# Henning1/resql

Measured on AMD Instinct MI355X. Metric: TPC-H Q1 rows/s at SF10, higher is better.
Workload: dtype int64; 1 GPU; TPC-H Q1 over lineitem SF10 (59999996 rows, 7 columns, 38 B/row) resident in HBM, row-range sharded over 1 GPU(s); rows=59999996, rows_per_gpu=59999996, world_size=1, rccl_ranks_seen=1, backend=none (single process, single GPU), ranks=1, self_launched=False, parallelism=single GPU

## Files before the change

__graft_entry__.py:

```python
from __future__ import annotations

import os
import subprocess
import sys

ROOT = os.path.dirname(os.path.abspath(__file__))
if ROOT not in sys.path:
    sys.path.insert(0, ROOT)


def _prepopulate_kernel_cache() -> int:
    from resql_amd import engine, tpch
    ctx = engine.Context(device=-1)
    compiled = 0
    try:
        for plan in tpch.standard_plans(0.01):
            tabs = [ctx.table(t) for t in plan.tables]
            try:
                q = ctx.compile(plan, tabs)
                compiled += 1
                q.close()
            except engine.EngineError as e:
                if e.status != 3:
                    raise
# ... 103 lines not shown
                    continue
                os.environ.update(env, RSQ_DICT_SCANS="1")
                try:
                    tabs = [ctx.table(t) for t in (host if host is not None else stmt.tables)]
                    (ctx.sql_compile(stmt, tabs) if isinstance(stmt, str) else ctx.compile(stmt, tabs)).close()
                    for t in tabs:
                        t.close()
                    done += 1
                except engine.EngineError as e:
                    failed += e.status not in (2, 3)
                finally:
                    for k in list(env) + ["RSQ_DICT_SCANS"]:
                        os.environ.pop(k, None)
        elif kind == "dictjoin":
            import dictjoincases
            for i, (stmt, host, env) in enumerate(dictjoincases.warm_statements()):
                if i not in items:
                    continue
                for sw in ("2", "1", "0"):
                    if sw == "2":
                        os.environ.update(env)
                    os.environ["RSQ_DICT_SCANS"] = sw
                    try:
                        tabs = [ctx.table(t) for t in host]
                        (ctx.sql_compile(stmt, tabs) if isinstance(stmt, str) else ctx.compile(stmt, tabs)).close()
                        for t in tabs:
                            t.close()
                        done += 1
                    except engine.EngineError as e:
                        failed += e.status not in (2, 3)
                    finally:
                        for k in list(env) + ["RSQ_DICT_SCANS"]:
                            os.environ.pop(k, None)
        elif kind == "resulttext":
            import resulttextcases
            for i, (sql, host) in enumerate(resulttextcases.warm_statements()):
                if i not in items:
                    continue
                try:
                    tabs = [ctx.table(t) for t in host]
                    ctx.sql_compile(sql, tabs).close()
                    for t in tabs:
                        t.close()
                    done += 1
                except engine.EngineError as e:
                    failed += e.status not in (2, 3)
        else:
            if kind == "fuzz":
                import fuzzplans
                make = lambda s: fuzzplans.make(s)[0]
            else:
                import test_gpu_fuzz_joins
                make = lambda s: test_gpu_fuzz_joins.make(7000 + s)[0]
            for seed in items:
                try:
                    plan = make(seed)
                    tabs = [ctx.table(t) for t in plan.tables]
                    ctx.compile(plan, tabs).close()
                    for t in tabs:
                        t.close()
                    done += 1
                except engine.EngineError as e:
                    failed += e.status not in (2, 3)
    finally:
        ctx.close()
    return done, failed


def _prepopulate_test_kernels() -> int:
    import json
    n = max(1, min(16, os.cpu_count() or 1))
    jobs = []
    for kind, seeds in (("fuzz", list(range(320))), ("joins", list(range(120))), ("sql", list(range(45)) + list(range(200, 225))),
                        ("narrow", list(range(200))),
                        ("typed", list(range(32))),
                        ("ldsfold", list(range(32))),
                        ("dictgroup", list(range(64))),
                        ("dicttail", list(range(32))),
                        ("dictjoin", list(range(32))),
                        ("resulttext", list(range(32)))):
        for i in range(n):
            part = seeds[i::n]
            if part:
                jobs.append((kind, part))
    try:
        with open(os.path.join(ROOT, "tests", "golden", "sql_reference.json")) as f:
            gold = json.load(f)
        texts = [g["sql"] for g in gold["results"].values() if "refused" not in g]
        for i in range(n):
            if texts[i::n]:
                jobs.append(("sql", texts[i::n]))
    except Exception:
        pass
    import subprocess
    import time
    import signal
    deadline = time.time() + float(os.environ.get("RSQ_BUILD_WARM_SECONDS", "900"))
    env = dict(os.environ, RSQ_COMPILE_HELPERS="0")
    pending, running, done, failed, crashed = list(jobs), [], 0, 0, 0
    while pending or running:
        while pending and len(running) < n:
            kind, items = pending.pop()
            running.append(subprocess.Popen([sys.executable, os.path.abspath(__file__), "--warm", kind, json.dumps(items)], env=env,
                                            stdout=subprocess.PIPE, stderr=subprocess.DEVNULL, text=True, start_new_session=True))
        for pr in list(running):
            if pr.poll() is not None:
                out = pr.stdout.read().strip().split()
                if pr.returncode == 0 and len(out) >= 2 and out[-2].isdigit() and out[-1].isdigit():
                    done += int(out[-2]); failed += int(out[-1])
                else:
                    crashed += 1
                running.remove(pr)
        if time.time() > deadline:
# ... 108 lines not shown
```

include/resql_hip.h:

```cpp
#ifndef RESQL_HIP_H
#define RESQL_HIP_H

#include "resql_plan.h"

#ifdef __cplusplus
extern "C" {
#endif

typedef struct rsq_ctx   rsq_ctx;
typedef struct rsq_table rsq_table;
typedef struct rsq_query rsq_query;

enum rsq_status {
    RSQ_OK = 0,
    RSQ_ERR_INVALID = 1,
    RSQ_ERR_TYPE = 2,
    RSQ_ERR_UNSUPPORTED = 3,
    RSQ_ERR_DEVICE = 4,
    RSQ_ERR_RUNTIME = 5,
    RSQ_ERR_NOMEM = 6
};

typedef struct rsq_config {
    uint32_t struct_size;
// ... 137 lines not shown
int  rsq_query_report(const rsq_query* q, rsq_report* out);
int  rsq_query_kernel_time_stats(rsq_query* q, double* sum_ms, uint64_t* executions, int32_t reset);
int  rsq_query_nested_loops_slices(const rsq_query* q, int32_t* out);
#define RSQ_NLJ_MIN_SLICE_ROWS 512
int32_t rsq_nested_loops_slices(int64_t base_workgroups, int64_t max_workgroups, int64_t inner_rows, int32_t configured);
const char* rsq_query_source(const rsq_query* q);
const char* rsq_query_explain(const rsq_query* q);
void rsq_query_destroy(rsq_query* q);

char* rsq_serialize_expr(rsq_ctx* ctx, const rsq_plan_desc* plan, int32_t expr, int32_t derive,
                         rsq_table* const* tables, int32_t n_tables);
char* rsq_result_serialize(const rsq_result_view* view);
void  rsq_free(void* p);
typedef struct rsq_result_text_options {
    uint32_t struct_size;
    int32_t  mode;
    int64_t  chunk_rows;
    int64_t  max_device_bytes;
} rsq_result_text_options;
enum rsq_text_fallback { RSQ_TEXT_FALLBACK_NONE = 0, RSQ_TEXT_FALLBACK_NO_DEVICE = 1, RSQ_TEXT_FALLBACK_SCHEMA = 2, RSQ_TEXT_FALLBACK_DOES_NOT_FIT = 3 };
typedef struct rsq_result_text_report {
    uint32_t struct_size;
    int32_t  path;
    int32_t  fallback_reason;
    int32_t  tuples_from_device;
    int64_t  rows, text_bytes, chunks;
    double   upload_ms, kernel_ms, download_ms, total_ms;
} rsq_result_text_report;
int  rsq_query_result_text(rsq_query* q, const rsq_result_text_options* options , rsq_result_text_report* report ,
                           char** text, int64_t* text_bytes);
int  rsq_query_result_write(rsq_query* q, const char* path, const rsq_result_text_options* options, rsq_result_text_report* report);
int  rsq_ctx_set_result_text(rsq_ctx* ctx, int32_t where);
int  rsq_ctx_set_row_cells(rsq_ctx* ctx, int32_t mode);
int  rsq_ctx_set_order_limit(rsq_ctx* ctx, int32_t where);
enum rsq_order_limit_fallback { RSQ_ORDER_LIMIT_FALLBACK_NONE = 0, RSQ_ORDER_LIMIT_FALLBACK_SHAPE = 1, RSQ_ORDER_LIMIT_FALLBACK_FEW_ROWS = 2,
                                RSQ_ORDER_LIMIT_FALLBACK_OVERFLOW = 3, RSQ_ORDER_LIMIT_FALLBACK_TIES = 4 };
typedef struct rsq_order_limit_report {
    uint32_t struct_size;
    int32_t  planned;
    int32_t  path;
    int32_t  fallback_reason;
    int32_t  first_key_column;
    int32_t  key_is32;
    int32_t  descending;
    int32_t  reserved;
    int64_t  rows, want, candidates, capacity;
    double   select_ms, copy_ms, tail_ms;
} rsq_order_limit_report;
int  rsq_query_order_limit_report(const rsq_query* q, rsq_order_limit_report* out);
int   rsq_ref_emission_order(const uint64_t* hashes, int64_t n, uint64_t min_size, int32_t parallel, uint32_t* out);
int   rsq_ref_emission_order_device(rsq_ctx* ctx, const uint64_t* hashes, int64_t n, uint64_t min_size, uint32_t* out);

int   rsq_prim_exclusive_scan(rsq_ctx* ctx, const uint32_t* counts, int64_t n, int32_t form, uint64_t* offsets , uint32_t* notes);
int   rsq_prim_rank_index(rsq_ctx* ctx, uint32_t* blocks , int64_t n_blocks, int32_t form,
                          uint32_t* chunk_base , uint32_t* notes);
int   rsq_prim_rank_place(rsq_ctx* ctx, const uint32_t* blocks , int64_t n_blocks, int64_t bm_min, int64_t bm_bits,
                          const int64_t* records , const uint32_t* used , int32_t n_waves,
                          int32_t region, int32_t n_words, int64_t capacity, int64_t* words_out , uint32_t* notes);
int   rsq_prim_radix_sort_pairs(rsq_ctx* ctx, const uint64_t* keys , const uint32_t* vals , int64_t n, int32_t key_bits,
                                uint64_t* keys_out , uint32_t* vals_out , uint32_t* notes);
int   rsq_prim_running_min(rsq_ctx* ctx, const int64_t* in , int64_t n, int64_t* out , uint32_t* notes);
int   rsq_prim_merge_group_rows(rsq_ctx* ctx, const int64_t* rows , int64_t n, int32_t stride, int32_t n_tab,
                                const int32_t* key_word, const int32_t* key_type, const int32_t* key_len, int32_t n_keys, const int32_t* acc_word,
                                const int32_t* acc_kind, int32_t n_acc, int64_t* out_rows , uint64_t* out_count, uint32_t* notes);
int   rsq_prim_topk_select(rsq_ctx* ctx, const int64_t* rows , int64_t n_rows, int64_t rows_upper_bound, int32_t stride,
                           int32_t key_word, int32_t is32, int32_t desc, int64_t want, int32_t form, const uint64_t* image_range ,
                           int64_t capacity, int64_t* cand_out , uint32_t* cand_count, uint32_t* notes);
int   rsq_prim_column_topk(rsq_ctx* ctx, const void* key , int32_t key_width, int64_t n, int32_t desc, int64_t want,
                           int64_t capacity, const void* payload , int32_t payload_width,
                           uint32_t* positions_out , void* payload_out , uint64_t* cand_count,
                           uint64_t* threshold_image, uint32_t* notes);
int   rsq_table_read_image(rsq_ctx* ctx, const rsq_table* t, const char* column, int32_t which, void* host_dst, size_t bytes, int64_t info[4]);

typedef struct rsq_sql_plan rsq_sql_plan;
int  rsq_sql_plan_select(rsq_ctx* ctx, const char* sql, rsq_table* const* tables, int32_t n_tables, rsq_sql_plan** out);
const rsq_plan_desc* rsq_sql_plan_desc(const rsq_sql_plan* plan);
void rsq_sql_plan_destroy(rsq_sql_plan* plan);
char* rsq_sql_plan_text(const rsq_sql_plan* plan);
int  rsq_sql_compile(rsq_ctx* ctx, const char* sql, rsq_table* const* tables, int32_t n_tables, rsq_query** out);
char* rsq_sql_describe(rsq_ctx* ctx, const char* sql, int32_t what);

typedef struct rsq_db rsq_db;
int  rsq_db_create(rsq_ctx* ctx, rsq_db** out);
int  rsq_db_execute(rsq_db* db, const char* sql, int32_t* kind, rsq_result_view* result);
const char* rsq_db_message(const rsq_db* db);
int  rsq_db_adopt_table(rsq_db* db, rsq_table* table);
int  rsq_db_report(const rsq_db* db, rsq_report* out);
int  rsq_db_load_report(const rsq_db* db, rsq_tbl_load_report* out);
int  rsq_db_result_text_report(const rsq_db* db, rsq_result_text_report* out);
int  rsq_db_order_limit_report(const rsq_db* db, rsq_order_limit_report* out);
void rsq_db_destroy(rsq_db* db);

enum rsq_merge_mode { RSQ_MERGE_AUTO = 0, RSQ_MERGE_RCCL = 1, RSQ_MERGE_PEER_COPY = 2 };
typedef struct rsq_multi_config {
    uint32_t struct_size;
    int32_t n_devices;
    const rsq_config* base;
    const int32_t* devices;
    int32_t merge;
    int32_t reserved0;
} rsq_multi_config;
typedef struct rsq_multi rsq_multi;
typedef struct rsq_multi_query rsq_multi_query;
int  rsq_multi_create(const rsq_multi_config* cfg, rsq_multi** out);
void rsq_multi_destroy(rsq_multi* m);
// ... 25 lines not shown
```

integration/resql_hip_binding.h:

```cpp
#pragma once

#include <map>
#include <memory>
#include <string>
#include <vector>
#include <cstring>

#include "resql_hip.h"

namespace resql_hip {

struct HipError : public ResqlError {
    int status;
    HipError(int st, const std::string& m) : ResqlError(m), status(st) {}
};

inline rsq_type toRsqType(SqlType t) {
    rsq_type r{(int32_t)t.tag, 0, 0, 0};
    if (t.tag == SqlType::DECIMAL) { r.precision = t.decimalSpec().precision; r.scale = t.decimalSpec().scale; }
    if (t.tag == SqlType::CHAR) r.len = (int32_t)t.charSpec().num;
    if (t.tag == SqlType::VARCHAR) r.len = (int32_t)t.varcharSpec().num;
    return r;
}

// ... 120 lines not shown
        c.print_assembly = cfg.printAssembly; c.print_flounder = cfg.printFlounder; c.print_performance = cfg.printPerformance;
        c.num_threads = cfg.numThreads; c.emit_machine_code = cfg.emitMachineCode; c.optimize = cfg.optimizeFlounder;
        c.device = device;
        int rc = rsq_ctx_create(&c, &ctx_);
        if (rc != RSQ_OK) throw HipError(rc, rsq_last_error(nullptr));
        report.config = cfg;
    }
    ~JitContextHip() {
        for (auto& kv : tables_) rsq_table_destroy(kv.second.t);
        if (ctx_) rsq_ctx_destroy(ctx_);
    }

    rsq_table* deviceTable(Relation* rel, const std::string& name) {
        auto it = tables_.find(rel);
        if (it == tables_.end()) {
            Resident r;
            r.t = fromBlocks(rel, name, 0, 0);
            noteSynced(rel, r);
            tables_[rel] = r;
            return r.t;
        }
        Resident& r = it->second;
        if (r.deviceOnly || rel->tupleNum() == r.tuples) return r.t;
        if (rel->tupleNum() < r.tuples) throw ResqlError("Relation " + name + " holds fewer tuples than its device copy.");
        rsq_table* more = fromBlocks(rel, name, r.blocks ? r.blocks - 1 : 0, r.blocks ? r.lastBlockBytes : 0);
        int rc = rsq_table_append(r.t, more);
        if (rc != RSQ_OK) { rsq_table_destroy(more); check(rc); }
        noteSynced(rel, r);
        return r.t;
    }

    void setRowstoreBridge(int where) { check(rsq_ctx_set_rowstore_bridge(ctx_, where)); }
    void setOrderLimit(int where) { check(rsq_ctx_set_order_limit(ctx_, where)); }

    int64_t bulkInsert(Relation* rel, const std::string& name, const std::string& fileName, char fieldTerminator) {
        std::vector<rsq_column> cols = columnsOf(rel);
        rsq_table_desc d{};
        std::strncpy(d.name, name.c_str(), RSQ_SYMBOL_MAX - 1);
        d.n_cols = (int32_t)cols.size(); d.cols = cols.data();
        rsq_table* t = nullptr;
        check(rsq_table_load_tbl(ctx_, &d, fileName.c_str(), fieldTerminator, 0, &t));
        const int64_t inserted = rsq_table_rows(t);
        auto it = tables_.find(rel);
        if (it == tables_.end()) {
            if (rel->tupleNum() != 0) { rsq_table_destroy(t); throw ResqlError("Table " + name + " holds host tuples: BULK INSERT onto the device needs an empty or device-resident table."); }
            Resident r; r.t = t; r.deviceOnly = true;
            tables_[rel] = r;
        } else {
            int rc = rsq_table_append(it->second.t, t);
            if (rc != RSQ_OK) { rsq_table_destroy(t); check(rc); }
        }
        return inserted;
    }

    std::unique_ptr<Relation> run(RelOperator* root, bool requestAll) {
        PlanDescriber pd;
        bool hasLimit = false; int64_t limit = 0;
        int rootIdx = pd.op(root, &hasLimit, &limit);
        rsq_plan_desc plan{};
        plan.exprs = pd.exprs.data(); plan.n_exprs = (int32_t)pd.exprs.size();
        plan.ops = pd.ops.data(); plan.n_ops = (int32_t)pd.ops.size();
        plan.root = rootIdx; plan.request_all = requestAll ? 1 : 0;
        plan.has_limit = hasLimit ? 1 : 0; plan.limit = limit;
        std::vector<rsq_table*> tabs;
        for (size_t i = 0; i < pd.tables.size(); i++) tabs.push_back(deviceTable(pd.tables[i], pd.tableNames[i]));
        rsq_query* q = nullptr;
// ... 62 lines not shown
```

resql_amd/csrc/aot_kernels.hip:

```cpp
#include <hip/hip_runtime.h>

#include <algorithm>
#include <cstring>

#include "engine_internal.h"
#include "scan_device.h"

namespace rsq {

template <typename T>
__global__ void __launch_bounds__(256) k_minmax(const T* __restrict__ p, i64 n, i64* out ) {
    i64 mn = 0x7fffffffffffffffll, mx = (i64)0x8000000000000000ull;
    u64 desc = 0;
    u64 same = 0;
    for (i64 i = blockIdx.x * (i64)blockDim.x + threadIdx.x; i < n; i += (i64)gridDim.x * blockDim.x) {
        i64 v = (i64)p[i];
        mn = v < mn ? v : mn; mx = v > mx ? v : mx;
        if (i > 0) { const i64 pv = (i64)p[i - 1]; if (v < pv) desc++; if (v == pv) same++; }
    }
    for (int m = 32; m >= 1; m >>= 1) {
        i64 a = __shfl_xor(mn, m, 64), b = __shfl_xor(mx, m, 64);
        mn = a < mn ? a : mn; mx = b > mx ? b : mx;
        desc += (u64)__shfl_xor((long long)desc, m, 64);
        same += (u64)__shfl_xor((long long)same, m, 64);
    }
    if ((threadIdx.x & 63) == 0) {
        atomicMin(&out[0], mn); atomicMax(&out[1], mx);
        if (desc) atomicAdd(reinterpret_cast<u64*>(&out[2]), desc);
        if (same) atomicAdd(reinterpret_cast<u64*>(&out[3]), same);
    }
}

__global__ void __launch_bounds__(256) k_byteset(const unsigned char* __restrict__ p, i64 n, unsigned* out ) {
    __shared__ unsigned s[8];
    if (threadIdx.x < 8) s[threadIdx.x] = 0;
    __syncthreads();
    unsigned loc[8] = {0, 0, 0, 0, 0, 0, 0, 0};
    for (i64 i = blockIdx.x * (i64)blockDim.x + threadIdx.x; i < n; i += (i64)gridDim.x * blockDim.x) {
// ... 17 lines not shown
        if (c.type.tag == RSQ_BOOL || (c.type.tag == RSQ_CHAR && c.type.len == 1)) {
            bool seen[256] = {false};
            const unsigned char* p = (const unsigned char*)c.dptr;
            for (int64_t i = 0; i < t.nRows; i++) seen[p[i]] = true;
            for (int v = 0; v < 256; v++) if (seen[v]) c.stats.distinctBytes.push_back((uint8_t)v);
            c.stats.min = c.stats.distinctBytes.front(); c.stats.max = c.stats.distinctBytes.back();
            c.stats.valid = true;
        } else if (rangeStatsType(c.type)) {
            int64_t mn = INT64_MAX, mx = INT64_MIN, prev = INT64_MIN;
            bool asc = true, strict = true;
            for (int64_t i = 0; i < t.nRows; i++) {
                int64_t v = (w == 8) ? ((const int64_t*)c.dptr)[i]
                          : (c.type.tag == RSQ_DATE ? (int64_t)((const uint32_t*)c.dptr)[i] : (int64_t)((const int32_t*)c.dptr)[i]);
                mn = std::min(mn, v); mx = std::max(mx, v);
                if (v < prev) asc = false;
                if (i > 0 && v <= prev) strict = false;
                prev = v;
            }
            c.stats.min = mn; c.stats.max = mx; c.stats.valid = true; c.stats.ascending = asc; c.stats.strictlyAscending = asc && strict;
        }
    }
}

int narrowWidth(const TableColumn& c) {
    if (!sw::flag<sw::RSQ_NARROW_SCANS>()) return 0;
    if (!c.owned || !c.dptr || !c.stats.valid || c.type.isString()) return 0;
    const int tag = c.type.tag;
    if (tag != RSQ_INT && tag != RSQ_BIGINT && tag != RSQ_DECIMAL && tag != RSQ_DATE) return 0;
    if (c.stats.min == INT64_MIN || c.stats.max == INT64_MAX || c.stats.max < c.stats.min) return 0;
    const uint64_t range = (uint64_t)c.stats.max - (uint64_t)c.stats.min;
    const int w = range <= 0xffull ? 1 : range <= 0xffffull ? 2 : range <= 0xffffffffull ? 4 : 0;
    if (tag == RSQ_INT && w != 1) return 0;
    return w > 0 && w < columnWidth(c.type) ? w : 0;
}

enum { DICT_MAX = 256, DICT_SLOTS = 1024, DICT_SAMPLE_ROWS = 65536, DICT_COLLECT_GRID = 512 };

__device__ inline unsigned dictHash(const unsigned char* p, int W) {
    unsigned h = 2166136261u;
    for (int i = 0; i < W; i++) h = (h ^ p[i]) * 16777619u;
    return h;
}
__device__ inline bool dictSame(const unsigned char* a, const unsigned char* b, int W) {
    for (int i = 0; i < W; i++) if (a[i] != b[i]) return false;
    return true;
}

__global__ void __launch_bounds__(256) k_dict_collect(const unsigned char* __restrict__ col, i64 n, int W, const unsigned* __restrict__ countsIn,
                                                      unsigned char* __restrict__ out, unsigned* __restrict__ counts, unsigned* overflow) {
    __shared__ unsigned long long slot[DICT_SLOTS];
    __shared__ unsigned cnt, wpos;
    for (int i = threadIdx.x; i < DICT_SLOTS; i += 256) slot[i] = ~0ull;
    if (threadIdx.x == 0) { cnt = 0; wpos = 0; }
    __syncthreads();
    for (i64 base = (i64)blockIdx.x * 256; base < n; base += (i64)gridDim.x * 256) {
        if (*(volatile unsigned*)&cnt > (unsigned)DICT_MAX || *(volatile unsigned*)overflow) break;
        const i64 r = base + threadIdx.x;
        if (r >= n) continue;
        if (countsIn && (unsigned)(r & 255) >= countsIn[r >> 8]) continue;
        const unsigned char* v = col + r * W;
        unsigned h = dictHash(v, W) & (DICT_SLOTS - 1);
        for (int probe = 0; probe < DICT_SLOTS; probe++, h = (h + 1) & (DICT_SLOTS - 1)) {
            unsigned long long cur = *(volatile unsigned long long*)&slot[h];
            if (cur == ~0ull) {
                cur = atomicCAS(&slot[h], ~0ull, (unsigned long long)r);
                if (cur == ~0ull) { if (atomicAdd(&cnt, 1u) >= (unsigned)DICT_MAX) atomicExch(overflow, 1u); break; }
// ... 263 lines not shown
    TableColumn& c = t.cols[(size_t)col];
    if (ctx.device < 0 || c.dictN <= 0 || !c.codePtr || !c.dictPtr || t.nRows <= 0) failInvalid("column " + c.name + " of table " + t.name + " has no dictionary codes on a device");
    if (which != 0 && which != 1) failInvalid("dictionary pass: 0 (recode) or 1 (encode)");
    RSQ_HIP(hipSetDevice(ctx.device));
    unsigned char ident[256];
    for (int i = 0; i < 256; i++) ident[i] = (unsigned char)i;
    unsigned char* dLut = (unsigned char*)ctx.alloc(256 + 16);
    unsigned* dFlag = (unsigned*)(dLut + 256);
    float ms = 0;
    unsigned notFound = 0;
    try {
        RSQ_HIP(hipMemcpyAsync(dLut, ident, 256, hipMemcpyHostToDevice, ctx.stream));
        RSQ_HIP(hipMemsetAsync(dFlag, 0, sizeof(unsigned), ctx.stream));
        RSQ_HIP(hipEventRecord(ctx.ev0, ctx.stream));
        if (which == 0) {
            const i64 vectors = ((i64)t.nRows + 15) >> 4;
            hipLaunchKernelGGL(k_dict_recode, dim3((unsigned)std::min<i64>(2048, (vectors + 255) / 256)), dim3(256), 0, ctx.stream, (unsigned char*)c.codePtr, (i64)t.nRows,
                               (const unsigned char*)dLut);
        } else {
            hipLaunchKernelGGL(k_dict_encode, dim3((unsigned)std::min<int64_t>(2048, (t.nRows + 255) / 256)), dim3(256), 0, ctx.stream, (const unsigned char*)c.dptr, (i64)t.nRows,
                               columnWidth(c.type), (const unsigned char*)c.dictPtr, c.dictN, (unsigned char*)c.codePtr, dFlag);
        }
        RSQ_HIP(hipGetLastError());
        RSQ_HIP(hipEventRecord(ctx.ev1, ctx.stream));
        RSQ_HIP(hipMemcpyAsync(&notFound, dFlag, sizeof notFound, hipMemcpyDeviceToHost, ctx.stream));
        RSQ_HIP(hipStreamSynchronize(ctx.stream));
        RSQ_HIP(hipEventElapsedTime(&ms, ctx.ev0, ctx.ev1));
    } catch (...) { (void)hipStreamSynchronize(ctx.stream); ctx.free(dLut); throw; }
    ctx.free(dLut);
    if (notFound) throw Error(RSQ_ERR_DEVICE, "dictionary pass over table " + t.name + ": a row holds a value that is not in the column's dictionary");
    return (double)ms;
}

template <typename T, typename N>
__global__ void __launch_bounds__(256) k_encode(const T* __restrict__ src, N* __restrict__ dst, i64 n, i64 base) {
    for (i64 i = blockIdx.x * (i64)blockDim.x + threadIdx.x; i < n; i += (i64)gridDim.x * blockDim.x)
        dst[i] = (N)((u64)(i64)src[i] - (u64)base);
}

template <typename T>
static void launchEncode(Context& ctx, const TableColumn& c, i64 n) {
    const unsigned grid = 1024;
    if (c.nw == 1) hipLaunchKernelGGL((k_encode<T, unsigned char>), dim3(grid), dim3(256), 0, ctx.stream, (const T*)c.dptr, (unsigned char*)c.nptr, n, (i64)c.nbase);
    else if (c.nw == 2) hipLaunchKernelGGL((k_encode<T, unsigned short>), dim3(grid), dim3(256), 0, ctx.stream, (const T*)c.dptr, (unsigned short*)c.nptr, n, (i64)c.nbase);
    else hipLaunchKernelGGL((k_encode<T, unsigned>), dim3(grid), dim3(256), 0, ctx.stream, (const T*)c.dptr, (unsigned*)c.nptr, n, (i64)c.nbase);
}

static void buildNarrowImages(Context& ctx, Table& t) {
    bool moved = false, launched = false;
    for (auto& c : t.cols) {
        const int w = t.nRows > 0 ? narrowWidth(c) : 0;
        const int64_t base = w ? c.stats.min : 0;
        const size_t bytes = w ? (((size_t)t.nRows * (size_t)w + 15) & ~(size_t)15) : 0;
        const bool keep = ctx.device >= 0 && c.nptr && w == c.nw && base == c.nbase && bytes == c.nbytes;
        if (!keep && c.nptr) { if (ctx.device >= 0) { ctx.freeRaw(c.nptr); ctx.columnImageBytes -= c.nbytes; } c.nptr = nullptr; moved = true; }
        c.nw = w; c.nbase = base; c.nbytes = bytes;
        if (!w || ctx.device < 0) continue;
        if (!c.nptr) { c.nptr = ctx.allocRaw(bytes); ctx.columnImageBytes += bytes; }
        launched = true;
        if (c.type.tag == RSQ_INT) launchEncode<int>(ctx, c, (i64)t.nRows);
        else if (c.type.tag == RSQ_DATE) launchEncode<unsigned>(ctx, c, (i64)t.nRows);
        else launchEncode<i64>(ctx, c, (i64)t.nRows);
    }
    if (launched) { RSQ_HIP(hipGetLastError()); RSQ_HIP(hipStreamSynchronize(ctx.stream)); }
    if (moved) t.layoutVersion++;
    buildDictImages(ctx, t);
}

void computeColumnStats(Context& ctx, Table& t) {
    if (ctx.device < 0) { hostStats(t); buildNarrowImages(ctx, t); return; }
    if (t.nRows == 0) {
        for (auto& c : t.cols) c.stats = ColumnStats();
        buildNarrowImages(ctx, t);
        return;
    }
    RSQ_HIP(hipSetDevice(ctx.device));
    i64* dmm = (i64*)ctx.alloc(4 * sizeof(i64));
    unsigned* dset = (unsigned*)ctx.alloc(8 * sizeof(unsigned));
    const unsigned grid = 1024;
    for (auto& c : t.cols) {
        c.stats = ColumnStats();
        if (!c.dptr) continue;
        if (c.type.tag == RSQ_BOOL || (c.type.tag == RSQ_CHAR && c.type.len == 1)) {
// ... 1357 lines not shown
```

resql_amd/csrc/api.cpp:

```cpp
#include <algorithm>
#include <chrono>
#include <cstdlib>
#include <cstring>
#include <map>
#include <thread>

#include "engine.h"
#include "sqlfront.h"
#include "hostref.h"

using namespace rsq;

namespace {
thread_local std::string g_createError;

template <typename F>
int guarded(Context* ctx, F&& f) {
    try { f(); return RSQ_OK; }
    catch (const Error& e) { if (ctx) ctx->lastError = e.what(); else g_createError = e.what(); return e.status; }
    catch (const std::bad_alloc&) { if (ctx) ctx->lastError = "out of host memory"; return RSQ_ERR_NOMEM; }
    catch (const std::exception& e) { if (ctx) ctx->lastError = e.what(); else g_createError = e.what(); return RSQ_ERR_INVALID; }
}

Context* C(rsq_ctx* c) { return reinterpret_cast<Context*>(c); }
// ... 405 lines not shown
    if (!ctx || !t || !name || !host_dst) return RSQ_ERR_INVALID;
    return guarded(C(ctx), [&] {
        const Table* tb = reinterpret_cast<const Table*>(t);
        int ci = tb->findCol(name);
        if (ci < 0 || !tb->cols[(size_t)ci].dptr) failInvalid(std::string("no such column: ") + name);
        size_t have = (size_t)tb->nRows * (size_t)columnWidth(tb->cols[(size_t)ci].type);
        if (bytes > have) failInvalid("read beyond the column");
        if (C(ctx)->device >= 0) RSQ_HIP(hipMemcpy(host_dst, tb->cols[(size_t)ci].dptr, bytes, hipMemcpyDeviceToHost));
        else memcpy(host_dst, tb->cols[(size_t)ci].dptr, bytes);
    });
}

int rsq_table_read_image(rsq_ctx* ctx, const rsq_table* t, const char* name, int32_t which, void* host_dst, size_t bytes, int64_t info[4]) {
    if (!ctx || !t || !name || !info || which < 0 || which > 2 || (bytes && !host_dst)) return RSQ_ERR_INVALID;
    return guarded(C(ctx), [&] {
        const Table* tb = reinterpret_cast<const Table*>(t);
        if (tb->ctx != C(ctx)) failInvalid("the table belongs to another context");
        int ci = tb->findCol(name);
        if (ci < 0) failInvalid(std::string("no such column: ") + name);
        const TableColumn& c = tb->cols[(size_t)ci];
        info[0] = c.nw; info[1] = c.nw ? c.nbase : 0; info[2] = c.dictN; info[3] = tb->nRows;
        if (!bytes) return;
        const bool device = C(ctx)->device >= 0;
        if (!device && which != 1) failUnsupported("a compile-only context keeps no narrow image and no dictionary codes");
        const size_t have = which == 0 ? (size_t)tb->nRows * (size_t)c.nw
                          : which == 1 ? (size_t)c.dictN * (size_t)columnWidth(c.type)
                                       : (c.dictN ? (size_t)tb->nRows : 0);
        if (bytes > have) failInvalid("read beyond the image");
        if (!device) { memcpy(host_dst, c.dict.data(), bytes); return; }
        const void* src = which == 0 ? c.nptr : which == 1 ? c.dictPtr : c.codePtr;
        if (!src) failInvalid("the column has no such image");
        RSQ_HIP(hipStreamSynchronize(C(ctx)->stream));
        RSQ_HIP(hipMemcpy(host_dst, src, bytes, hipMemcpyDeviceToHost));
    });
}

void rsq_table_destroy(rsq_table* t) { delete T(t); }

int rsq_query_compile(rsq_ctx* ctx, const rsq_plan_desc* plan, rsq_table* const* tables, int32_t n_tables, rsq_query** out) {
    if (!ctx || !plan || !out || n_tables < 0) return RSQ_ERR_INVALID;
    *out = nullptr;
    return guarded(C(ctx), [&] {
        std::unique_ptr<QueryHandle> h(new QueryHandle{C(ctx), nullptr});
        h->q = compileQuery(*C(ctx), *plan, tables, n_tables);
        *out = reinterpret_cast<rsq_query*>(h.release());
    });
}

#define QH(q) reinterpret_cast<QueryHandle*>(q)

int rsq_query_execute(rsq_query* q) {
    if (!q) return RSQ_ERR_INVALID;
    return guarded(QH(q)->ctx, [&] { executeQuery(*QH(q)->q, false); });
}

int rsq_query_await_kernels(rsq_query* q) {
    if (!q) return RSQ_ERR_INVALID;
    return guarded(QH(q)->ctx, [&] { awaitKernels(*QH(q)->q); });
}

int rsq_query_execute_partial(rsq_query* q, void** dev_ptr, int64_t* n_min_words, int64_t* n_max_words, int64_t* n_sum_words) {
    if (!q || !dev_ptr || !n_min_words || !n_max_words || !n_sum_words) return RSQ_ERR_INVALID;
    return guarded(QH(q)->ctx, [&] {
        executeQuery(*QH(q)->q, true);
        partialBuffer(*QH(q)->q, dev_ptr, n_min_words, n_max_words, n_sum_words);
    });
// ... 852 lines not shown
```

resql_amd/csrc/codegen.cpp:

```cpp
#include "codegen_internal.h"

namespace rsq {
namespace cg {

void Walker::addArg(const std::string& name, const std::string& ctype, uint64_t v) {
    for (auto& a : pipe.args) if (a.name == name) return;
    pipe.args.push_back({name, ctype, v});
}

void Walker::produce(OpNode* o, std::vector<std::string> request) {
    switch (o->tag) {
        case RSQ_OP_SCAN: produceScan(o, request); break;
        case RSQ_OP_SELECTION: {
            o->schema.clear();
            std::vector<std::string> r = request;
            requiredAttributes(o->exprs[0], r);
            requestOf[o] = request;
            produce(o->child[0], r);
            break;
        }
        case RSQ_OP_PROJECTION: {
            std::vector<std::string> r;
            for (Expr* e : o->exprs) requiredAttributes(e, r);
            produce(o->child[0], r);
            break;
        }
        case RSQ_OP_HASHJOIN: {
            requestOf[o] = request;
            std::vector<std::string> all = request;
            for (Expr* e : o->exprs) requiredAttributes(e, all);
            joinPhase[o] = 1;
            produce(o->child[0], all);
            joinPhase[o] = 2;
            produce(o->child[1], all);
            break;
        }
        case RSQ_OP_AGGREGATION: {
            if (q.agg) failUnsupported("more than one aggregation in a plan");
            q.agg = o;
            std::vector<std::string> r;
// ... 135 lines not shown
        for (auto& b : numeric) line(b.ct + " " + b.var + "_b[" + Bs + "]; rsq::nlj_ld_block<" + b.ct + ", " + Bs + ">(a." + b.cn + ", " + N + "_jb, " + b.var + "_b);");
        line("#pragma unroll");
        openScope("for (int " + N + "_u = 0; " + N + "_u < " + Bs + "; " + N + "_u++) {");
        line("const i64 " + N + "_j = " + N + "_jb + " + N + "_u;");
        body += pairDeep.substr(0, pairDeep.find('\n') + 1);
        for (auto& b : numeric) line("const " + b.ct + " " + b.var + " = " + b.var + "_b[" + N + "_u];");
        body += pairDeep.substr(pairDeep.find('\n') + 1);
        closeScope();
        closeScope();
        openScope("for (i64 " + N + "_j = " + N + "_jb; " + N + "_j != " + hi + "; " + N + "_j++) {");
        body += pairFlat.substr(0, pairFlat.find('\n') + 1);
        singleLoads();
        body += pairFlat.substr(pairFlat.find('\n') + 1);
        closeScope();
    }
    closeScope();
}

Schema Walker::prune(const Schema& s, const std::vector<std::string>& req) {
    Schema r;
    for (auto& a : s) if (has(req, a.name)) r.push_back(a);
    return r;
}

void Walker::produceScan(OpNode* o, std::vector<std::string> request) {
    Table* t = o->table;
    if (o->derived >= 0) nameDerivedColumns(q, o);
    if (q.requestAll) request.clear();
    pipe = Pipeline();
    pipe.src = t;
    pipe.unroll = 1;
    pipe.blockThreads = 256;
    pipe.maxGrid = q.maxGrid;
    colTypes.clear(); colIsString.clear(); colNarrow.clear(); colDict.clear(); colTyped.clear(); eg.typedLeaves.clear(); nDictTables = 0; rowParams.clear(); rowArgsTail.clear(); rowArgsTailGuarded.clear(); bitmapPrefetch.clear();
    body.clear(); stateDecl.clear(); stateInit.clear(); prologue.clear(); epilogue.clear(); fileScope.clear(); helperFns.clear();
    explainSteps.clear(); indent = 1; matchSlotTable = -1; slotVar.clear(); symbolOrigin.clear(); symbolWord.clear();
    multiMatchAbove = false; repeatedKeysAbove.clear(); denseRefusal.clear();
    selective = false; compacted = false; stage2Body.clear(); cqLive.clear();
    leadCond.clear(); leadCols.clear(); leadPass = 1.0; leadPassComplete = true;
    pairSplit = std::string::npos; pairCond.clear();
    strPrefetch.clear(); strPrefetchWidth.clear(); strStaged.clear(); strStagedBytes = 0; postTile.clear(); foldTile.clear(); accRegs = 0; eg.strWordVars.clear();
    eg.symbols.clear();
    o->schema.clear();
    const bool narrowScans = sw::flag<sw::RSQ_NARROW_SCANS>();
    for (size_t ci = 0; ci < t->cols.size(); ci++) {
        const TableColumn& c = t->cols[ci];
        if (!request.empty() && !has(request, c.name)) continue;
        if (!c.dptr && !t->derived) {
            if (request.empty()) continue;
            failInvalid("column " + c.name + " is needed by the plan but was declared without data");
        }
        int k = (int)pipe.cols.size();
        pipe.cols.push_back((int)ci);
        std::string var = "v_" + std::to_string(k);
        eg.symbols[c.name] = Sym{var, c.type};
        symbolOrigin[c.name] = -1;
        o->schema.push_back({c.name, c.type});
        pipe.bytesPerRow += columnWidth(c.type);
        const int nw = (!t->derived && c.owned && narrowScans && !c.type.isString() && (c.nptr || q.ctx.device < 0)) ? c.nw : 0;
        colNarrow.push_back(nw);
        const bool dictCoded = !t->derived && c.owned && c.type.isString() && c.dictN > 0 && sw::dictScansEnabled() && (c.codePtr || q.ctx.device < 0);
        colDict.push_back(dictCoded ? c.type.len : 0);
        pipe.storedBytesPerRow += dictCoded ? 1 : nw ? nw : columnWidth(c.type);
        if (dictCoded) {
            const std::string K = std::to_string(k);
            addArg("c" + K, "const u8*", (uint64_t)(uintptr_t)c.codePtr);
            addArg("d" + K, "const char*", (uint64_t)(uintptr_t)c.dictPtr);
            addArg("dn" + K, "i64", (uint64_t)c.dictN);
            colIsString.push_back(0); colTypes.push_back("u8");
            rowParams += ", u8 vc_" + K;
            rowArgsTail += ", a.c" + K + "[r]";
            rowArgsTailGuarded += ", (valid ? a.c" + K + "[r] : (u8)0)";
            line("const rsq::Str " + var + " = " + dictDecode(k, "vc_" + K) + ";");
        } else if (c.type.isString()) {
            addArg("c" + std::to_string(k), "const char*", (uint64_t)(uintptr_t)c.dptr);
            colIsString.push_back(1); colTypes.push_back("");
            line("const rsq::Str " + var + " = rsq::str(a.c" + std::to_string(k) + " + lr * " + std::to_string(c.type.len) + ", " +
                 std::to_string(c.type.len) + ");");
        } else {
            std::string ct = ExprGen::ctype(c.type);
            if (nw) {
                addArg("c" + std::to_string(k), std::string("const ") + (nw == 1 ? "u8" : nw == 2 ? "u16" : "u32") + "*", (uint64_t)(uintptr_t)c.nptr);
                addArg("fb" + std::to_string(k), "i64", (uint64_t)c.nbase);
            } else addArg("c" + std::to_string(k), "const " + ct + "*", (uint64_t)(uintptr_t)c.dptr);
            colIsString.push_back(0); colTypes.push_back(ct);
            rowParams += ", " + ct + " " + var;
            rowArgsTail += ", " + colAt(k, "r");
            rowArgsTailGuarded += ", (valid ? " + colAt(k, "r") + " : (" + ct + ")0)";
        }
    }
    explainSteps.push_back("scan " + t->name + " [" + (t->derived ? std::string("rows of this execution") : std::to_string((long long)t->nRows) + " rows") + ", " +
                           std::to_string((long long)pipe.bytesPerRow) + " B/row" +
                           (pipe.storedBytesPerRow != pipe.bytesPerRow ? ", " + std::to_string((long long)pipe.storedBytesPerRow) + " B/row stored" : std::string()) + "]");
    consume(o->parent, o);
    finishPipeline();
}

bool Walker::sideRange(const Expr* e, double& lo, double& hi, int& col) {
    if (e->tag == RSQ_E_TYPECAST && e->child) {
        if (!sideRange(e->child, lo, hi, col)) return false;
        const int ds = (e->type.tag == RSQ_DECIMAL ? e->type.scale : 0) - (e->child->type.tag == RSQ_DECIMAL ? e->child->type.scale : 0);
        const double f = std::pow(10.0, (double)ds);
        lo *= f; hi *= f;
        return true;
    }
    auto linear = [&](double v) -> double {
        if (e->type.tag != RSQ_DATE) return v;
        const int64_t d = (int64_t)v;
        return (double)((d / 10000) * 372 + ((d / 100) % 100 - 1) * 31 + (d % 100 - 1));
    };
    if (e->tag == RSQ_E_CONSTANT && !e->type.isString()) { lo = hi = linear((double)e->ival); col = -1; return true; }
    if ((e->tag == RSQ_E_ADD || e->tag == RSQ_E_SUB) && e->child && e->child->next && e->type.tag != RSQ_DATE) {
        double alo, ahi, blo, bhi; int ac = -1, bc = -1;
        if (!sideRange(e->child, alo, ahi, ac) || !sideRange(e->child->next, blo, bhi, bc) || ac >= 0 || bc >= 0) return false;
        const int s0 = e->type.tag == RSQ_DECIMAL ? e->type.scale : 0;
        const double fa = std::pow(10.0, (double)(s0 - (e->child->type.tag == RSQ_DECIMAL ? e->child->type.scale : 0)));
        const double fb = std::pow(10.0, (double)(s0 - (e->child->next->type.tag == RSQ_DECIMAL ? e->child->next->type.scale : 0)));
        lo = hi = e->tag == RSQ_E_ADD ? alo * fa + blo * fb : alo * fa - blo * fb; col = -1;
        return true;
    }
    if (e->tag == RSQ_E_ATTRIBUTE) {
        auto so = symbolOrigin.find(e->symbol);
        if (so == symbolOrigin.end() || so->second != -1) return false;
        const int ci = pipe.src->findCol(e->symbol);
        if (ci < 0 || !pipe.src->cols[(size_t)ci].stats.valid || pipe.src->cols[(size_t)ci].type.isString()) return false;
        lo = linear((double)pipe.src->cols[(size_t)ci].stats.min); hi = linear((double)pipe.src->cols[(size_t)ci].stats.max); col = ci;
// ... 344 lines not shown
```

resql_amd/csrc/codegen_agg.cpp:

```cpp
#include "codegen_internal.h"
#include "row_cells.h"

namespace rsq {
namespace cg {

void Walker::collectAccumulators(OpNode* o) {
    for (Expr* g : o->exprs2) q.pool.addId(g);
    for (Expr* s : o->splitAgg) q.pool.addId(s);
    q.accums.clear(); q.splitToAccum.clear();
    q.accums.push_back(Accum{RSQ_E_MIN, "#firstrow", "row", Type(RSQ_BIGINT), 2});
    for (Expr* s : o->splitAgg) {
        Accum ac; ac.kind = s->tag; ac.type = s->type;
        dictTablesWithin(s);
        switch (s->tag) {
            case RSQ_E_COUNT: ac.key = "COUNT"; ac.input = eg.emit(s); ac.merge = 0; ac.inputExpr = nullptr; break;
            case RSQ_E_SUM:
                if (s->type.tag != RSQ_DECIMAL && s->type.tag != RSQ_BIGINT) failType("ADD code generation not implemented for datatype");
                ac.key = "SUM" + structuralKey(s->child); ac.input = eg.emit(s); ac.merge = 0; ac.inputExpr = s->child; break;
            case RSQ_E_MIN: case RSQ_E_MAX:
                if (s->type.tag != RSQ_DECIMAL && s->type.tag != RSQ_BIGINT && s->type.tag != RSQ_DATE)
                    failType(s->tag == RSQ_E_MAX ? "ADD code generation not implemented for datatype" : "LESS_THAN code generation not implemented for datatype");
                ac.key = std::string(s->tag == RSQ_E_MIN ? "MIN" : "MAX") + structuralKey(s->child);
                ac.input = "((i64)(" + eg.emit(s) + "))"; ac.merge = s->tag == RSQ_E_MIN ? 2 : 3; ac.inputExpr = s->child; break;
            default: failType("Aggregation type not implemented in updateAggregates(..).");
// ... 684 lines not shown
    for (int w = 1; w < W; w++) k << (w > 1 ? " : " : "") << (w < W - 1 ? "w == " + std::to_string(w) + " ? " : "") << "(i64)" << q.accumSlot[(size_t)w];
    k << ";\n        if (g < " << D << ") a.out[blk * " << D << " + g] = s_tab[i];\n    }\n}\n";
    pipe.sourceStagedAgg = k.str();
}

bool Walker::envelopeOf(const TableColumn& c, bool& neg, int& bits) {
    if (!c.owned || !c.stats.valid || c.stats.min <= -(int64_t(1) << 40) || c.stats.max >= (int64_t(1) << 40)) return false;
    const uint64_t m = (uint64_t)std::max(c.stats.max < 0 ? -c.stats.max : c.stats.max, c.stats.min < 0 ? -c.stats.min : c.stats.min);
    bits = 0;
    while (bits < 63 && (m >> bits) != 0) bits++;
    neg = c.stats.min < 0;
    return true;
}

bool Walker::typeScanColumns() {
    if (!sw::flag<sw::RSQ_NARROW_SCANS>() || compacted || !pipe.src || pipe.src->derived) return false;
    colTyped.assign(colTypes.size(), 0);
    std::string widen;
    for (size_t k = 0; k < colTypes.size(); k++) {
        if (colIsString[k] || coded((int)k) || !colNarrow[k] || colTypes[k] != "i64") continue;
        bool neg = false; int bits = 0;
        if (!envelopeOf(pipe.src->cols[(size_t)pipe.cols[k]], neg, bits) || bits > 31) continue;
        const std::string K = std::to_string(k);
        auto patch = [&](std::string& text, const std::string& from, const std::string& to) {
            for (size_t at = 0; (at = text.find(from, at)) != std::string::npos; at += to.size()) {
                const size_t end = at + from.size();
                if (isdigit((unsigned char)from.back()) && end < text.size() && isdigit((unsigned char)text[end])) { at = end - to.size(); continue; }
                text.replace(at, from.size(), to);
            }
        };
        patch(rowParams, ", i64 v_" + K, ", i32 n_" + K);
        patch(rowArgsTail, "rsq::dec<i64>(a.c" + K + "[", "rsq::dec<i32>(a.c" + K + "[");
        patch(rowArgsTailGuarded, "rsq::dec<i64>(a.c" + K + "[", "rsq::dec<i32>(a.c" + K + "[");
        colTyped[k] = 1; colTypes[k] = "i32";
        eg.typedLeaves["v_" + K] = ExprGen::TypedLeaf{"n_" + K, neg, bits};
        widen += "    const i64 v_" + K + " = (i64)n_" + K + "; (void)v_" + K + ";\n";
    }
    if (widen.empty()) return false;
    body = widen + body;
    return true;
}

void Walker::emitDenseAggregation(OpNode* o) {
    const int64_t D = q.denseGroups;
    const int W = (int)q.accums.size();
    line("const int gid = " + groupIdExpr() + ";");
    const bool typed = q.aggMode == AggMode::DENSE_REG && typeScanColumns();
    auto emitInputs = [&](const std::vector<char>& part32) {
        for (int w = 1; w < W; w++) {
            const Accum& ac = q.accums[(size_t)w];
            const std::string name = "in" + std::to_string(w);
            if (typed && ac.merge == 0 && ac.inputExpr && eg.pureArithmetic(ac.inputExpr)) {
                const ExprGen::TV v = eg.emitTyped(ac.inputExpr);
                if (v.is32 && part32[(size_t)w]) line("const i32 " + name + " = " + v.text + ";");
                else line("const i64 " + name + " = " + ExprGen::wide(v) + ";");
            } else line("const i64 " + name + " = " + ac.input + ";");
        }
    };
    if (q.aggMode != AggMode::DENSE_REG) emitInputs(std::vector<char>((size_t)W, 0));
    const bool fr32 = typed && !underNestedLoops() && pipe.src->nRows < (int64_t)0xffffffffll && pipe.src->totalRows() < (int64_t)0xffffffffll;
    auto inOf = [&](int w) { return w == 0 ? std::string("row") : "in" + std::to_string(w); };
    addArg("out", "u64*", 0);
    std::ostringstream ep;
    if (q.aggMode == AggMode::DENSE_REG) {
        std::vector<char> part32((size_t)W, 0);
        std::vector<rowcells::Accumulator> envelopes((size_t)W, rowcells::Accumulator{false, false, -1});
// ... 335 lines not shown
```

resql_amd/csrc/codegen_internal.h:

```cpp
#pragma once
#include <algorithm>
#include <cmath>
#include <cstring>
#include <functional>
#include <set>
#include <sstream>

#include "engine_internal.h"


namespace rsq {
namespace cg {


struct Sym { std::string var; Type type; };


struct ExprGen {
    std::map<std::string, Sym> symbols;
    std::map<std::string, int> strWordVars;
    bool int16Cast = false;
    std::map<const Expr*, std::string> tabled;

    static std::string ctype(const Type& t) {
// ... 258 lines not shown
            close += ")";
        }
        if (c) out += "(" + emit(c) + ")";
        else out += (e->type.isString() ? std::string("rsq::str(\"\", 0)") : "((" + ctype(e->type) + ")0)");
        return out + close;
    }
};

inline std::string fromWord(const std::string& w, const Type& t) {
    switch (t.tag) {
        case RSQ_BIGINT: case RSQ_DECIMAL: return w;
        case RSQ_INT: case RSQ_DATE: return "((i32)(" + w + "))";
        case RSQ_BOOL: return "((u8)(" + w + "))";
        case RSQ_CHAR: if (t.len == 1) return "((u8)(" + w + "))"; [[fallthrough]];
        case RSQ_VARCHAR: return "rsq::str_from_addr(" + w + ", " + std::to_string(t.len) + ")";
        default: failUnsupported("value type cannot be carried in a hash table word");
    }
}
inline std::string toWord(const std::string& v, const Type& t) {
    if (t.isString()) return "rsq::str_addr(" + v + ")";
    return "((i64)(" + v + "))";
}

struct Walker {
    Query& q;
    ExprGen eg;

    Pipeline pipe;
    std::vector<std::string> colTypes;
    std::vector<int> colIsString;
    std::vector<int> colNarrow;
    std::string colAt(int k, const std::string& r) const {
        const std::string K = std::to_string(k);
        if (k < (int)colNarrow.size() && colNarrow[(size_t)k]) return "rsq::dec<" + colTypes[(size_t)k] + ">(a.c" + K + "[" + r + "], a.fb" + K + ")";
        return "a.c" + K + "[" + r + "]";
    }
    std::string tileLoad(int k, const std::string& dst) const {
        const std::string K = std::to_string(k);
        if (k < (int)colNarrow.size() && colNarrow[(size_t)k]) return "rsq::ld2n(a.c" + K + " + b, a.fb" + K + ", " + dst + ");";
        return "rsq::ld2(a.c" + K + " + b, " + dst + ");";
    }
    std::vector<int> colDict;
    std::vector<char> colTyped;
    bool typedCol(int k) const { return k >= 0 && k < (int)colTyped.size() && colTyped[(size_t)k] != 0; }
    static bool envelopeOf(const TableColumn& c, bool& neg, int& bits);
    bool typeScanColumns();
    bool coded(int k) const { return k >= 0 && k < (int)colDict.size() && colDict[(size_t)k] != 0; }
    std::string paramName(int k) const { return (coded(k) ? "vc_" : typedCol(k) ? "n_" : "v_") + std::to_string(k); }
    std::string dictDecode(int k, const std::string& code) const {
        const std::string K = std::to_string(k), W = std::to_string(colDict[(size_t)k]);
        return "rsq::str(a.d" + K + " + (u32)(" + code + ") * " + W + "u, " + W + ")";
    }
    int nDictTables = 0;
    int dictTableColumn(const Expr* e, int col = -1);
    void dictTablesWithin(Expr* e);
    int storedWidth(int k) const {
        if (k < (int)colNarrow.size() && colNarrow[(size_t)k]) return colNarrow[(size_t)k];
        return colTypes[(size_t)k] == "i64" ? 8 : colTypes[(size_t)k] == "i32" ? 4 : 1;
    }
    std::string rowParams, rowArgsTail, rowArgsTailGuarded;
    struct BitmapPrefetch { std::string first; int second; bool interleaved; };
    std::vector<BitmapPrefetch> bitmapPrefetch;
    std::string body;
    std::string closers;
    std::string stateDecl, stateInit, prologue, epilogue, fileScope;
    std::string helperFns;
    std::vector<std::string> explainSteps;
    int indent = 1;
    int matchSlotTable = -1;
    std::map<int, std::string> slotVar;
    std::map<std::string, int> symbolOrigin;
    std::map<std::string, int> symbolWord;
    bool multiMatchAbove = false;
    std::string repeatedKeysAbove;
    std::string denseRefusal;
    bool underNestedLoops() const { return !q.nljs.empty(); }
    bool selective = false, compacted = false;
    std::string leadCond; std::vector<int> leadCols; double leadPass = 1.0;
    std::string stage2Prefix;
    struct CompFilter { std::string table, symbol, stage2Var; int64_t bits; };
    std::vector<CompFilter> compFilters;
    bool inStage2 = false;
    bool leadPassComplete = true;
    size_t pairSplit = std::string::npos; std::string pairCond;
    std::string stage2Body;
    std::vector<std::pair<std::string, Sym>> cqLive;

    explicit Walker(Query& q_) : q(q_) { eg.int16Cast = jitInt16Cast(q_.ctx); }

    void line(const std::string& s) { body += std::string((size_t)indent * 4, ' ') + s + "\n"; }
    void openScope(const std::string& head) { line(head); indent++; }
    void closeScope() { indent--; line("}"); }
    void addArg(const std::string& name, const std::string& ctype, uint64_t v);

    void produce(OpNode* o, std::vector<std::string> request);

    std::map<OpNode*, std::vector<std::string>> requestOf;
    std::map<OpNode*, int> joinPhase;

    static bool has(const std::vector<std::string>& v, const std::string& s) { return std::find(v.begin(), v.end(), s) != v.end(); }

    Schema prune(const Schema& s, const std::vector<std::string>& req);

    void produceScan(OpNode* o, std::vector<std::string> request);

    bool sideRange(const Expr* e, double& lo, double& hi, int& col);
    double passFraction(const Expr* e);
    void leadColumnsOf(const Expr* e, std::vector<int>& out, bool& ok);
    std::vector<std::pair<int, int>> strPrefetch;
    std::map<int, int> strPrefetchWidth;
    std::string foldTile;
    int accRegs = 0;
    bool rowCells = false;
    static constexpr const char* RC_IFNOT = "\x01rc-ifnot\n"; static constexpr const char* RC_IF = "\x01rc-if\n";
    static constexpr const char* RC_ELSE = "\x01rc-else\n"; static constexpr const char* RC_END = "\x01rc-end\n";
    static void resolveRowCells(std::string& text, bool keep);
    std::string postTile;
    std::map<int, int> strStaged;
    int strStagedBytes = 0;
    void prefetchComparedStrings(const Expr* e);
    void noteLeadingSelection(const Expr* e, const std::string& cond);

    void consume(OpNode* o, OpNode* from);

    bool downstreamMaterializes(OpNode* o);
    bool compactThen(OpNode* o, const std::function<void()>& downstream);
// ... 79 lines not shown
```

resql_amd/csrc/codegen_loop.cpp:

```cpp
#include "codegen_internal.h"

namespace rsq {
namespace cg {

std::string Walker::postTileFor(const std::string& tile) {
    std::string out = postTile;
    for (size_t at; (at = out.find("$TILE")) != std::string::npos;) out.replace(at, 5, tile);
    return out;
}

void Walker::stagedChunkLoads(std::ostringstream& s, const std::string& ind, const char* pre, int col, int u) {
    const int W = strPrefetchWidth[col];
    for (int r = 0; r < stagedRounds(col); r++)
        s << ind << pre << col << "_" << u << "_" << r << " = rsq::ld_str_chunk<" << W << ", " << r << ">(a.c" << col << " + (b - lane * 2) * " << W << ", lane);\n";
}

void Walker::stagedUnstage(std::ostringstream& s, const std::string& ind, int u) {
    for (auto& sp : strPrefetch) {
        auto it = strStaged.find(sp.first);
        if (it == strStaged.end()) continue;
        const int W = strPrefetchWidth[sp.first];
        for (int r = 0; r < stagedRounds(sp.first); r++)
            s << ind << "rsq::st_str_chunk<" << W << ", " << r << ">(strt + " << it->second << ", lane, q" << sp.first << "_" << u << "_" << r << ");\n";
    }
// ... 9 lines not shown
    }
    if (!strStaged.empty()) s << ind << "rsq::wave_lds_order();\n";
}

void Walker::emitLateLoads(std::ostringstream& s, const std::string& tile, int u, const std::vector<char>& lateCol, const std::string& tileEnd) {
    s << "        if (" << tile << " < " << tileEnd << ") {\n";
    for (int j = 0; j < 2; j++) {
        s << "            const bool lp" << j << " = lead_pred(a";
        for (int k : leadCols) s << ", t" << k << "_" << u << "[" << j << "]";
        s << ");\n";
    }
    s << "            if (lp0 | lp1) {\n                const i64 b = ((" << tile << ") << 7) + lane * 2;\n";
    for (size_t k = 0; k < lateCol.size(); k++) if (lateCol[k]) s << "                " << tileLoad((int)k, "t" + std::to_string(k) + "_" + std::to_string(u)) << "\n";
    s << "            }\n        }\n";
}

void Walker::resolveRowCells(std::string& text, bool keep) {
    std::string out;
    bool drop = false;
    for (size_t at = 0; at < text.size();) {
        size_t end = text.find('\n', at);
        end = end == std::string::npos ? text.size() : end + 1;
        const std::string ln = text.substr(at, end - at);
        at = end;
        if (ln == RC_IFNOT) { if (keep) out += "#if !RSQ_ROW_CELLS\n"; }
        else if (ln == RC_IF) { if (keep) out += "#if RSQ_ROW_CELLS\n"; else drop = true; }
        else if (ln == RC_ELSE) { if (keep) out += "#else\n"; else drop = true; }
        else if (ln == RC_END) { if (keep) out += "#endif\n"; drop = false; }
        else if (!drop) out += ln;
    }
    text = out;
}

void Walker::finishPipeline() {
    while (indent > 1) closeScope();
    addArg("n_rows", "i64", (uint64_t)pipe.src->nRows);
    addArg("row0", "i64", (uint64_t)pipe.src->row0);
    addArg("err", "u32*", (uint64_t)(uintptr_t)q.ctx.dErr);
    if (pipe.gridPerCU == 2 && pipe.storedBytesPerRow > 0)
        pipe.unroll = (int)std::max<int64_t>(1, std::min<int64_t>(foldTile.empty() ? 4 : 2, (4608 + pipe.storedBytesPerRow * 128 - 1) / (pipe.storedBytesPerRow * 128)));
    if (pipe.compact) pipe.unroll = 4;
    const bool mat = pipe.sink == SinkKind::MATERIALIZE;
    std::ostringstream s;
    s << "// generated by resql_amd/csrc/codegen.cpp\n//   ";
    for (size_t i = 0; i < explainSteps.size(); i++) {
        std::string step = explainSteps[i];
        const size_t lb = step.find(" [");
        if (step.compare(0, 5, "scan ") == 0 && lb != std::string::npos) step = step.substr(0, lb);
        const size_t kb = step.find(", key bitmap of ");
        if (kb != std::string::npos) {
            const size_t ke = step.find(" bits", kb);
            if (ke != std::string::npos) step = step.substr(0, kb) + ", key bitmap" + step.substr(ke + 5);
        }
        s << (i ? " -> " : "") << step;
    }
    s << "\n";
    if (1) s << "#define RSQ_NT_LOADS 1\n";
    s << "#include \"rsq_device.h\"\n";
    s << fileScope;
    if (nDictTables) {
        s << "__shared__ u64 s_dt[" << 4 * nDictTables << "];      // truth tables over dictionary-coded columns: 256 bits each, filled in the kernel's prologue\n";
        prologue += "    __syncthreads();\n";
        pipe.extraLdsBytes += 32 * nDictTables;
    }
    const bool cq = pipe.compact;
    const bool dbgStamps = sw::num<sw::RSQ_DEBUG_TAIL>() != 0 && !(pipe.sink == SinkKind::AGGREGATE && q.aggMode == AggMode::DENSE_REG);
    if (dbgStamps) addArg("dbg", "u64*", 0);
    if (pipe.staged && (cq || mat || !bitmapPrefetch.empty() || !pipe.lazyCols.empty() ||
// ... 38 lines not shown
        if (fourWaves) { pipe.unroll = u; pipe.gridPerCU = 4; }
    }
    rowCells = rowCells && fourWaves && pipe.sink == SinkKind::AGGREGATE;
    for (std::string* text : {&stateDecl, &prologue, &body, &foldTile, &epilogue}) resolveRowCells(*text, rowCells);
    if (!rowCells) pipe.rowCellsEnvelopes.clear();
    const int U = pipe.unroll;
    if (strStagedBytes > 0) {
        pipe.extraLdsBytes += (pipe.blockThreads / 64) * strStagedBytes;
        prologue += "    __shared__ __attribute__((aligned(16))) char s_strt[(RSQ_BLOCK_THREADS / 64) * " + std::to_string(strStagedBytes) + "];\n    char* const strt = s_strt + (threadIdx.x >> 6) * " +
                    std::to_string(strStagedBytes) + ";\n";
    }
    const int NV = 1 + pipe.compactWords;
    const bool queuesLimit = (144 * 1024) / std::max(1, (pipe.blockThreads / 64) * NV * 192 * 8 + pipe.extraLdsBytes) < 4;
    const int QCAP = (queuesLimit ? 128 : 192);
    const int NVL = 1 + pipe.compactWordsLazy;
    const bool twoForms = !pipe.lazyCols.empty();
    if (cq) {
        const int ldsPerWG = (pipe.blockThreads / 64) * NV * QCAP * 8 + pipe.extraLdsBytes;
        const int ldsPerWGLazy = (pipe.blockThreads / 64) * NVL * QCAP * 8 + pipe.extraLdsBytes;
        const int wgCap = pipe.unroll >= 3 ? 6 : 8;
        pipe.gridPerCU = std::max(2, std::min(wgCap, (144 * 1024) / std::max(1, ldsPerWG)));
        pipe.gridPerCULazy = std::max(2, std::min(wgCap, (144 * 1024) / std::max(1, ldsPerWGLazy)));
        stateDecl += "    int cq_n = 0;\n    u32 cq_rows = 0;\n    i64* cq;\n";
        addArg("cq_total", "unsigned long long*", 0);
        epilogue += "    if (blockIdx.x < 64) {\n        const u64 v = rsq::wave_sum((u64)st.cq_rows);\n        if ((threadIdx.x & 63) == 0 && v) atomicAdd(a.cq_total, (unsigned long long)v);\n    }\n";
        const std::string nv = twoForms ? "RSQ_CQ_NV" : std::to_string(NV);
        prologue += "    __shared__ i64 s_cq[(RSQ_BLOCK_THREADS / 64) * " + nv + " * " + std::to_string(QCAP) + "];\n";
        prologue += "    st.cq = s_cq + (threadIdx.x >> 6) * " + nv + " * " + std::to_string(QCAP) + ";\n";
    }
    if (twoForms) s << "#if RSQ_LAZY\n#define RSQ_CQ_NV " << NVL << "\n#else\n#define RSQ_CQ_NV " << NV << "\n#endif\n";
    s << "#ifndef RSQ_BLOCK_THREADS\n#define RSQ_BLOCK_THREADS " << pipe.blockThreads << "\n#endif\n";
    if (fourWaves) s << "#define RSQ_MIN_WG 4\n";
    s << "struct Args {\n";
    for (auto& a : pipe.args) s << "    " << a.ctype << " " << a.name << ";\n";
    s << "};\nstruct State {\n" << stateDecl << "};\n";
    s << helperFns;
    if (cq) {
        s << "#ifdef RSQ_STAGE2_CALL\nstatic __device__ __attribute__((noinline)) void stage2(const Args& a, State& st, const i64 row";
        for (int k = 0; k < pipe.compactWords; k++) s << ", const i64 qw_" << k;
        s << ")\n#else\n";
        s << "static RSQ_DEV void stage2(const Args& a, State& st, const i64 row";
        for (int k = 0; k < pipe.compactWords; k++) s << ", const i64 qw_" << k;
        s << ")\n#endif\n{\n" << stage2Body << "}\n";
        pipe.hasStage2 = true;
        s << "static RSQ_DEV void cq_drain(const Args& a, State& st, const int count) {\n";
        s << "    const int lane = threadIdx.x & 63;\n    const int i = st.cq_n - count + lane;\n    rsq::wave_lds_order();      // (the entries were pushed by other lanes)\n";
        s << "    if (lane < count) {\n        stage2(a, st, st.cq[i]";
        for (int k = 0; k < pipe.compactWordsLazy; k++) s << ", st.cq[" << (k + 1) * QCAP << " + i]";
        if (pipe.compactWords > pipe.compactWordsLazy) {
            s << "\n#if RSQ_LAZY\n            ";
            for (int k = pipe.compactWordsLazy; k < pipe.compactWords; k++) s << ", 0";
            s << "\n#else\n            ";
            for (int k = pipe.compactWordsLazy; k < pipe.compactWords; k++) s << ", st.cq[" << (k + 1) * QCAP << " + i]";
            s << "\n#endif\n        ";
        }
        s << ");\n        st.cq_rows++;\n    }\n    st.cq_n -= count;\n}\n";
    }
    if (late) {
        s << "static RSQ_DEV bool lead_pred(const Args& a";
        for (int k : leadCols) s << ", " << colTypes[(size_t)k] << " " << paramName(k);
        s << ") { ";
        for (int k : leadCols) if (coded(k)) s << "const rsq::Str v_" << k << " = " << dictDecode(k, paramName(k)) << "; (void)v_" << k << "; ";
        for (int k : leadCols) if (typedCol(k)) s << "const i64 v_" << k << " = (i64)n_" << k << "; ";
        s << "return " << leadCond << "; }\n";
    }
    if (pipe.staged) s << "#if RSQ_AGG_VARIANT == 3\ntemplate <int SP_SLOT>       // the row's place among the rows a thread handles per round\n#endif\n";
    s << "static RSQ_DEV void row_fn(const Args& a, State& st, const i64 lr" << (cq ? ", const bool valid" : "") << rowParams << ") {\n";
// ... 265 lines not shown
        const bool eagerOk = cqPipelined && eagerRegs * U <= budget, lazyOk = cqPipelined && lazyRegs * U <= budget;
        if (latePipelined || regPipelined || (eagerOk && (lazyOk || pipe.lazyCols.empty()))) emitPipelinedLoop();
        else if (lazyOk && !pipe.lazyCols.empty()) { s << "#if RSQ_LAZY\n"; emitPipelinedLoop(); s << "#else\n"; emitPlainLoop(); s << "#endif\n"; }
        else emitPlainLoop();
    }
    if (dbgStamps) s << "    if (a.dbg && threadIdx.x == 0) a.dbg[(u64)blockIdx.x * 8 + 1] = (u64)wall_clock64();\n";
    if (!postTile.empty()) s << "    st.in_tile = false;\n";
    if (cq) {
        s << "    for (i64 rb = (ntiles << 7) + (i64)" << bx << " * blockDim.x; rb < a.n_rows; rb += (i64)" << gx << " * blockDim.x) {\n";
        s << "        const i64 r = rb + threadIdx.x;\n        const bool valid = r < a.n_rows;\n";
        s << "        row_fn(a, st, r, valid" << rowArgsTailGuarded << ");\n";
        s << "        while (st.cq_n >= 64) cq_drain(a, st, 64);\n    }\n";
        s << "    while (st.cq_n > 0) cq_drain(a, st, st.cq_n < 64 ? st.cq_n : 64);\n";
    } else {
        if (mat) {
            s << "    for (i64 rb = (ntiles << 7) + (i64)blockIdx.x * blockDim.x + (i64)(threadIdx.x & ~63u); rb < a.n_rows; rb += (i64)gridDim.x * blockDim.x) {\n";
            s << "        const i64 r = rb + lane;\n        const bool valid = r < a.n_rows;\n";
            s << "        const i64 ttile = ntiles + ((rb - (ntiles << 7)) >> 6);\n        const i64 slot = ttile * 64 + lane;\n";
            s << "#if RSQ_PASS == 2\n        st.pos = a.toffs[ttile] + (u64)rsq::wave_excl_sum_u32(valid ? a.cnt[slot] : 0u);\n#endif\n";
            s << "        if (valid) row_fn(a, st, r" << rowArgsTail << ");\n";
            s << "#if RSQ_PASS == 1\n        a.cnt[slot] = st.cnt;\n        { const u32 ts = (u32)rsq::wave_sum((u64)st.cnt); if (lane == 0) a.tcnt[ttile] = ts; }\n        st.cnt = 0;\n#endif\n";
            s << "    }\n";
        } else {
        s << "    for (i64 r = (ntiles << 7) + (i64)" << bx << " * blockDim.x + threadIdx.x; r < a.n_rows; r += (i64)" << gx << " * blockDim.x) {\n";
        s << "        row_fn(a, st, r" << rowArgsTail << ");\n";
        s << "    }\n";
        }
    }
    if (pipe.staged) s << "#endif\n";
    if (dbgStamps) s << "    if (a.dbg && threadIdx.x == 0) a.dbg[(u64)blockIdx.x * 8 + 2] = (u64)wall_clock64();\n";
    s << epilogue;
    if (dbgStamps) s << "    __syncthreads();\n    if (a.dbg && threadIdx.x == 0) a.dbg[(u64)blockIdx.x * 8 + 3] = (u64)wall_clock64();\n";
    s << "}\n";
    pipe.source = s.str();
    if (!pipe.lazyCols.empty()) pipe.source = "#define RSQ_LAZY 0\n" + pipe.source;
    if (mat) {
        pipe.sourcePass1 = "#define RSQ_PASS 1\n" + pipe.source;
        pipe.source = "#define RSQ_PASS 2\n" + pipe.source;
    }
    if (q.aggPad > 1 && pipe.sink == SinkKind::AGGREGATE && !pipe.partitioned) {
        pipe.sourceFlat = "#define RSQ_OUT_STRIDE 1\n" + pipe.source;
        pipe.source = "#define RSQ_OUT_STRIDE " + std::to_string(q.aggPad) + "\n" + pipe.source;
    }
    if (rowCells) {
        const std::string guard = "#ifndef RSQ_ROW_CELLS\n#define RSQ_ROW_CELLS 0\n#endif\n";
        pipe.sourceCells = "#define RSQ_ROW_CELLS 1\n" + guard + pipe.source;
        pipe.source = guard + pipe.source;
        if (!pipe.sourceFlat.empty()) { pipe.sourceFlatCells = "#define RSQ_ROW_CELLS 1\n" + guard + pipe.sourceFlat; pipe.sourceFlat = guard + pipe.sourceFlat; }
    }
    if (pipe.partitioned) {
        pipe.sourcePartCount = "#define RSQ_AGG_VARIANT 1\n#define RSQ_BLOCK_THREADS 1024\n" + pipe.source;
        pipe.sourcePartScatter = "#define RSQ_AGG_VARIANT 2\n#define RSQ_BLOCK_THREADS 1024\n" + pipe.source;
        if (pipe.staged) pipe.sourceStagedScatter = "#define RSQ_AGG_VARIANT 3\n#define RSQ_BLOCK_THREADS 1024\n" + pipe.source;
        pipe.source = "#define RSQ_AGG_VARIANT 0\n" + pipe.source;
    }
    if (!pipe.lazyCols.empty()) {
        pipe.sourceLazy = pipe.source;
        const std::string off = "#define RSQ_LAZY 0\n";
        const size_t at = pipe.sourceLazy.find(off);
        if (at == std::string::npos) pipe.sourceLazy.clear();
        else {
            const int minWg = 0;
            pipe.sourceLazy.replace(at, off.size(), "#define RSQ_LAZY 1\n" + (minWg ? "#define RSQ_MIN_WG " + std::to_string(minWg) + "\n" : std::string()));
        }
    }
    std::string ex = "pipeline " + std::to_string(q.pipelines.size()) + ": ";
    for (size_t i = 0; i < explainSteps.size(); i++) ex += (i ? " -> " : "") + explainSteps[i];
// ... 14 lines not shown
```

resql_amd/csrc/engine.cpp:

```cpp
#include <algorithm>
#include <atomic>
#include <chrono>
#include <cstring>
#include <functional>
#include <sstream>

#include "engine_internal.h"

namespace rsq {

namespace {

uint64_t inverseOdd64(uint64_t a) { uint64_t x = a; for (int i = 0; i < 6; i++) x *= 2 - a * x; return x; }

void buildOps(Query& q, const rsq_plan_desc& p) {
    int extra = 0;
    for (int i = 0; i < p.n_ops; i++) if (p.ops[i].tag == RSQ_OP_ORDERBY) extra++;
    for (int i = 0; i < p.n_ops + extra; i++) q.ops.emplace_back(new OpNode());
    int nextExtra = p.n_ops;
    for (int i = 0; i < p.n_ops; i++) {
        const rsq_op& d = p.ops[i];
        OpNode* o = q.ops[(size_t)i].get();
        o->tag = d.tag;
        if (d.n_exprs < 0 || d.n_exprs > RSQ_MAX_OP_EXPRS || d.n_exprs2 < 0 || d.n_exprs2 > RSQ_MAX_OP_EXPRS) failInvalid("bad expression count");
// ... 173 lines not shown
        for (int64_t g = 0; g < D; g++) init[(size_t)(q.accumSlot[w] * D + g)] = idv;
    }
    q.dAgg = (uint64_t*)q.ctx.alloc(words * 8);
    q.dAggInit = (uint64_t*)q.ctx.alloc(words * 8);
    RSQ_HIP(hipMemcpy(q.dAggInit, init.data(), words * 8, hipMemcpyHostToDevice));
    q.hAgg.assign(words, 0);
    q.pinnedWords = words;
    q.tableWords = words;
    if (q.aggPad > 1) {
        q.padWords = words * (size_t)q.aggPad;
        std::vector<uint64_t> pinit(q.padWords + 1, 0);
        for (size_t i = 0; i < words; i++) pinit[i * (size_t)q.aggPad] = init[i];
        q.dAggWork = (uint64_t*)q.ctx.alloc((q.padWords + 1) * 8);
        q.dAggWorkInit = (uint64_t*)q.ctx.alloc((q.padWords + 1) * 8);
        RSQ_HIP(hipMemcpy(q.dAggWorkInit, pinit.data(), (q.padWords + 1) * 8, hipMemcpyHostToDevice));
        q.pinnedWords = q.padWords;
    }
}

std::string tierSource(const Pipeline& p, const std::string& source, bool quick) {
    return quick && p.hasStage2 ? "#define RSQ_STAGE2_CALL 1\n" + source : source;
}
static std::vector<std::string> kernelSources(const Query& q, bool quick = false) {
    std::vector<std::string> v;
    for (auto& p : q.pipelines) {
        auto T = [&](const std::string& s) { return tierSource(p, s, quick); };
        if (!p.sourcePass1.empty()) v.push_back(T(p.sourcePass1));
        if (!p.sourceFlat.empty()) v.push_back(T(p.sourceFlat));
        if (p.partitioned) { v.push_back(T(p.sourcePartCount)); v.push_back(T(p.sourcePartScatter)); v.push_back(p.sourcePartAgg); }
        if (p.staged) { v.push_back(T(p.sourceStagedScatter)); v.push_back(p.sourceStagedAgg); }
        v.push_back(T(p.source));
        if (!p.sourceCells.empty()) v.push_back(T(p.sourceCells));
        if (!p.sourceFlatCells.empty()) v.push_back(T(p.sourceFlatCells));
        if (!p.sourceLazy.empty()) v.push_back(T(p.sourceLazy));
        if (p.ldsSlots > 64 && q.aggMode == AggMode::HASH && p.sink == SinkKind::AGGREGATE && q.aggTable >= 0) {
            v.push_back(T("#define RSQ_LC_SLOTS 64\n" + p.source));
            if (!p.sourceLazy.empty()) v.push_back(T("#define RSQ_LC_SLOTS 64\n" + p.sourceLazy));
        }
    }
    return v;
}
static void resolveKernels(Query& q, bool quick = false) {
    Context& ctx = q.ctx;
    ctx.compileManyToCache(kernelSources(q, quick));
    q.quickTier = quick;
    for (auto& p : q.pipelines) {
        auto T = [&](const std::string& s) { return tierSource(p, s, quick); };
        p.fewGroupKernels.clear();
        if (!p.sourcePass1.empty()) p.kernelPass1 = &ctx.getKernel(T(p.sourcePass1), p.entry);
        if (!p.sourceFlat.empty()) p.kernelFlat = &ctx.getKernel(T(p.sourceFlat), p.entry);
        if (p.partitioned) {
            p.kernelPartCount = &ctx.getKernel(T(p.sourcePartCount), p.entry);
            p.kernelPartScatter = &ctx.getKernel(T(p.sourcePartScatter), p.entry);
            p.kernelPartAgg = &ctx.getKernel(p.sourcePartAgg, "rsq_part_agg");
        }
        if (p.staged) {
            p.kernelStagedScatter = &ctx.getKernel(T(p.sourceStagedScatter), p.entry);
            p.kernelStagedAgg = &ctx.getKernel(p.sourceStagedAgg, "rsq_staged_agg");
        }
        p.kernel = &ctx.getKernel(T(p.source), p.entry);
        if (!p.sourceCells.empty()) p.kernelCells = &ctx.getKernel(T(p.sourceCells), p.entry);
        if (!p.sourceFlatCells.empty()) p.kernelFlatCells = &ctx.getKernel(T(p.sourceFlatCells), p.entry);
        if (!p.sourceLazy.empty()) p.kernelLazy = &ctx.getKernel(T(p.sourceLazy), p.entry);
        if (ctx.device < 0 && p.ldsSlots > 64 && q.aggMode == AggMode::HASH && p.sink == SinkKind::AGGREGATE && q.aggTable >= 0) {
            (void)ctx.getKernel("#define RSQ_LC_SLOTS 64\n" + p.source, p.entry);
            if (!p.sourceLazy.empty()) (void)ctx.getKernel("#define RSQ_LC_SLOTS 64\n" + p.sourceLazy, p.entry);
        }
    }
}


static uint64_t fnv1a64(const std::string& s, uint64_t h = 1469598103934665603ull) {
    for (unsigned char c : s) { h ^= c; h *= 1099511628211ull; }
    return h;
}
static std::string planMemoKey(const Query& q) {
    uint64_t h = 1469598103934665603ull;
    for (auto& p : q.pipelines) h = fnv1a64(p.source, h) * 0x9E3779B97F4A7C15ull;
    std::string k = std::to_string(h);
    if (q.maxGrid) k += "|g" + std::to_string(q.maxGrid);
    for (Table* t : q.tables) k += "|" + std::to_string(t->uid) + "." + std::to_string(t->version) + "." + std::to_string(t->nRows) + "." + std::to_string(t->row0) + "." + std::to_string(t->nRowsTotal);
    return k;
}

static void applyPlanMemo(Query& q) {
    Context& ctx = q.ctx;
    if (ctx.planMemoOff || ctx.device < 0 || q.genericActive) return;
    if (!q.derived.empty()) return;
    q.memoKey = planMemoKey(q);
    auto it = ctx.planMemo.find(q.memoKey);
    if (it == ctx.planMemo.end()) return;
    Context::PlanMemo& m = it->second;
    if (m.joins.size() != q.hashTables.size() || m.pipes.size() != q.pipelines.size()) return;
    m.stamp = ++ctx.planMemoClock;
    for (size_t i = 0; i < q.pipelines.size(); i++) {
// ... 1550 lines not shown
```

resql_amd/csrc/engine.h:

```cpp
#pragma once

#include <hip/hip_runtime.h>

#include <atomic>
#include <cstdint>
#include <cstdio>
#include <cstdlib>
#include <functional>
#include <map>
#include <tuple>
#include <memory>
#include <mutex>
#include <set>
#include <string>
#include <vector>

#include "expr.h"
#include "hostref.h"
#include "mempool.h"
#include "resql_hip.h"
#include "rowstore.h"
#include "switches.h"
#include "tbl.h"

#define RSQ_RANK_CHUNK_BLOCKS 1024

namespace rsq {

#define RSQ_HIP(call)                                                                              \
    do {                                                                                           \
        hipError_t _e = (call);                                                                    \
        if (_e != hipSuccess)                                                                      \
            throw ::rsq::Error(RSQ_ERR_DEVICE, std::string(#call) + ": " + hipGetErrorString(_e)); \
    } while (0)

struct ColumnStats {
    bool valid = false;
    int64_t min = 0, max = 0;
    bool ascending = false;
    bool strictlyAscending = false;
    std::vector<uint8_t> distinctBytes;
};

struct TableColumn {
    std::string name;
    Type type;
    void* dptr = nullptr;
    bool owned = false;
    ColumnStats stats;
    int nw = 0;
    int64_t nbase = 0;
    void* nptr = nullptr;
    size_t nbytes = 0;
    int dictN = 0;
    std::vector<uint8_t> dict;
    void* dictPtr = nullptr;
    void* codePtr = nullptr;
    size_t codeBytes = 0;
    bool dictShared = false;
};

int narrowWidth(const TableColumn& c);

struct Context;

inline std::atomic<uint64_t> g_nextTableUid{1};

struct Table {
    Context* ctx = nullptr;
    uint64_t uid = g_nextTableUid.fetch_add(1);
    uint64_t version = 0;
    void bumpVersion();
    uint64_t layoutVersion = 0;
    std::string name;
    bool derived = false;
    uint64_t derivedEstimate = 0;
    int64_t nRows = 0;
    int64_t row0 = 0;
    int64_t nRowsTotal = -1;
    std::vector<ColumnStats> ownStats;
    int64_t totalRows() const { return nRowsTotal >= 0 ? nRowsTotal : nRows; }
    const ColumnStats& shardStats(size_t col) const { return ownStats.empty() ? cols[col].stats : ownStats[col]; }
    std::vector<TableColumn> cols;
    int findCol(const std::string& n) const {
        for (size_t i = 0; i < cols.size(); i++) if (cols[i].name == n) return (int)i;
        return -1;
    }
    ~Table();
};

struct Kernel {
    hipModule_t module = nullptr;
    hipFunction_t fn = nullptr;
    bool fromCache = false;
    std::map<int, int> residentPerCU;
// ... 36 lines not shown
    std::vector<hipEvent_t> eventPool;
    hipEvent_t takeEvent();
    void giveEvent(hipEvent_t e) { if (e) eventPool.push_back(e); }
    std::unique_ptr<Arena> devArena, pinArena, pinNcArena;
    bool driverAlloc = false;
    size_t arenaKeepBytes = 0;
    struct AllocStats { uint64_t devCalls = 0, pinCalls = 0, rawCalls = 0; double devMs = 0, pinMs = 0, rawMs = 0; } allocStats;
    void setStream(hipStream_t s, bool callers);
    void* scratchAlloc(size_t bytes);
    void scratchFree(void* p);
    std::vector<std::pair<void*, size_t>> scratchFreeList, scratchLive;
    struct TailArena { void* dev = nullptr; size_t devBytes = 0; void* pinned = nullptr; size_t pinnedBytes = 0; };
    TailArena spareTailArena;
    ReplayScratch replayScratch;
    std::vector<uint32_t> replayOrder;
    struct PlanMemo {
        struct Join { int64_t buildRows = -1; bool dupKeys = false; uint32_t lastCount = 0; };
        struct Pipe { int64_t stage2Rows = -1; bool stagedExact = false; std::vector<uint32_t> stagedCaps; int64_t stagedCapsRows = -1; int cellsChoice = -1; };
        std::vector<Join> joins;
        std::vector<Pipe> pipes;
        int64_t hashCapacity = 0; uint32_t hashCount = 0; bool charGroupsNeedMerge = false;
        int64_t matLastTotal = -1;
        bool narrowRowsOff = false, fusedSelectOff = false, chainedIndexOff = false, scanChainedOff = false;
        uint32_t stageWorkgroups = 0;
        uint64_t stamp = 0;
    };
    std::map<std::string, PlanMemo> planMemo;
    struct KeyIndex { uint32_t* dBitmap = nullptr; int64_t bmBlocks = 0, bmMin = 0, bmBits = 0; int refs = 0; bool retired = false; uint64_t uid = 0; };
    typedef std::tuple<uint64_t, uint64_t, int64_t, int64_t, int> KeyIndexKey;
    std::map<KeyIndexKey, KeyIndex> keyIndexes;
    void retireKeyIndexes(uint64_t uid);
    void releaseKeyIndex(KeyIndex* k);
    uint64_t columnImageBytes = 0;
    uint64_t planMemoClock = 0, planMemoHits = 0;
    bool planMemoOff = false;
    int rowCellsMode = -1;
    bool shardCompile = false;
    int32_t resultText = 0;
    int32_t rowstoreBridge = 0;
    int32_t orderLimit = 0;
};

rsq_config readConfig(const rsq_config* cfg, bool multiBase = false);
inline bool jitInt16Cast(const Context& c) { return (c.cfg.compat_flags & RSQ_COMPAT_JIT_INT16_CAST) != 0; }

void launch(Context& ctx, Kernel& k, unsigned grid, unsigned block, const std::vector<uint64_t>& args);

void computeColumnStats(Context& ctx, Table& t);
void generateTable(Context& ctx, Table& t, int kind, int64_t row0, int64_t nRows, double sf, int64_t param, uint64_t seed);
double measureReadBandwidth(Context& ctx, size_t bytes, int iters);
size_t scanTempBytes(int64_t n);
void exclusiveScanCounts(Context& ctx, const uint32_t* counts, uint64_t* offs, int64_t n, void* temp, size_t tempBytes);
void exclusiveScanCountsChained(Context& ctx, const uint32_t* counts, uint64_t* offs, int64_t n, void* temp, size_t tempBytes);
void fillU64Async(Context& ctx, uint64_t* dptr, size_t n, uint64_t value);
struct FillItem { void* p; size_t bytes; uint64_t value; };
void publishStatusAsync(Context& ctx, uint64_t* hostWords, const uint32_t* err, const uint32_t* groupCount, const uint32_t* candCount,
                        const uint64_t* pipeStats, int nPipelines, const int64_t* rows = nullptr, int rowWords = 0, uint32_t maxInline = 0,
                        int64_t* hostRows = nullptr,
                        const uint64_t* word3 = nullptr,
                        const uint64_t* copySrc = nullptr, uint64_t* copyDst = nullptr, uint32_t copyWords = 0);
void fillBatchAsync(Context& ctx, const FillItem* items, int count);
void rankTableIndex(Context& ctx, uint32_t* bitmap, int64_t nBlocks, uint32_t* chunkTotal, uint32_t* chunkBase);
void rankTableIndexChained(Context& ctx, uint32_t* bitmap, int64_t nBlocks, uint32_t* chain, uint32_t* chunkBase);
void rankTablePlace(Context& ctx, const int64_t* temp, const uint32_t* used, uint32_t nWaves, uint32_t region, const uint32_t* nRecords, int nWords,
                    const uint32_t* bitmap, int64_t bmMin, int64_t bmBits, const uint32_t* chunkBase, int64_t nBlocks, int64_t* words,
                    int64_t capacity);
// ... 149 lines not shown
```

resql_amd/csrc/engine_internal.h:

```cpp
#pragma once

#include <atomic>
#include <chrono>
#include <cstdarg>
#include <cstdio>
#include <deque>
#include <thread>
#include <map>
#include <memory>
#include <string>
#include <vector>

#include "engine.h"
#include "hostref.h"
#include "dense_groups.h"
#include "row_cells.h"

namespace rsq {

struct Attr { std::string name; Type type; };
typedef std::vector<Attr> Schema;
int schemaTupleSize(const Schema& s);
int schemaOffset(const Schema& s, const std::string& name);

// ... 56 lines not shown
    const Table* directSrc = nullptr;
    bool rankCapable = false;
    bool setOnly = false;
    bool bmInterleaved = false;
    bool rank = false;
    int64_t* dTemp = nullptr;
    uint32_t* dTempUsed = nullptr;
    int64_t tempWaves = 0, tempRegion = 0;
    uint32_t* dChunkTotal = nullptr;
    uint32_t* dChunkBase = nullptr;
    int64_t bmBlocks = 0;
    std::vector<int> derefCodes;
    std::vector<int> derefCondTables;
    int compactStride = 0;
    int* dDeref = nullptr;
    int64_t buildRows = -1;
    bool dupKeys = false;
    bool prepared = false;
};

struct Accum {
    int kind;
    std::string key;
    std::string input;
    Type type;
    int merge;
    Expr* inputExpr = nullptr;
};


enum class AggMode { NONE, DENSE_REG, DENSE_LDS_PRIVATE, DENSE_LDS_SHARED, DENSE_GLOBAL, AT_JOIN_ENTRY, HASH };
enum class SinkKind { AGGREGATE, BUILD, MATERIALIZE };

struct ArgSlot { std::string name; std::string ctype; uint64_t value; };

struct GenericInstr { uint8_t op, dst, a, b; uint32_t c; int64_t imm; };
enum GenericOp : uint8_t { G_COL = 1, G_CONST, G_ADD, G_SUB, G_MUL, G_DIV, G_LT, G_LE, G_GT, G_GE, G_EQ, G_NE, G_AND, G_OR, G_MULI, G_DIVI,
                           G_SELECT, G_FILTER };
enum { G_MAX_COLS = 16, G_MAX_KEYS = 4, G_MAX_ACCS = 16, G_MAX_SET = 16, G_REGS = 32, G_MAX_INSTR = 256 };
struct GenericProgram {
    std::vector<GenericInstr> code;
    struct Col { const void* ptr; int kind; };
    std::vector<Col> cols;
    struct Key { int reg; int byteSet; int64_t min, card, stride; uint8_t values[G_MAX_SET]; int nValues; };
    std::vector<Key> keys;
    struct Acc { int reg; int merge; int64_t block; };
    std::vector<Acc> accs;
};
enum GenericOp2 : uint8_t { G_COLADDR = 32, G_CONSTADDR, G_MOV, G_CAST16, G_STREQ, G_LIKE, G_STRWORD, G_PROBE };
enum { G2_REGS = 40, G2_MAX_COLS = 24, G2_MAX_TABLES = 8, G2_MAX_KEYW = 40, G2_MAX_DEPTH = 4, G2_MAX_OUT = 24, G2_MAX_ACCS = 16, G2_MAX_KEYS = 4, G2_MAX_SET = 32,
       G2_MAX_PAYLOAD = 24, G2_MAX_CHARKEYS = 8 };
enum { G2_SINK_BUILD = 1, G2_SINK_DENSE, G2_SINK_ENTRY, G2_SINK_HASH, G2_SINK_MATERIALIZE };
struct GenericProbeDesc {
    int32_t table, nKeys, nPayload, slotReg, single;
    uint8_t keyReg[8]; uint8_t payloadReg[G2_MAX_PAYLOAD];
};
struct GenericSinkDesc {
    int32_t kind, table, nKeys, nPayload, slotReg, nAccs, nOut, nCharKeys;
    uint8_t keyReg[G2_MAX_KEYW];
    uint8_t wordStr[G2_MAX_KEYW], wordOff[G2_MAX_KEYW], wordN[G2_MAX_KEYW];
    uint8_t payloadReg[G2_MAX_PAYLOAD];
    int32_t accReg[G2_MAX_ACCS], accMerge[G2_MAX_ACCS], accBlock[G2_MAX_ACCS];
    int32_t keyByteSet[G2_MAX_KEYS], keyNValues[G2_MAX_KEYS]; int64_t keyMin[G2_MAX_KEYS], keyCard[G2_MAX_KEYS], keyStride[G2_MAX_KEYS];
    uint8_t keyValues[G2_MAX_KEYS][G2_MAX_SET];
    uint8_t charFirst[G2_MAX_CHARKEYS], charLast[G2_MAX_CHARKEYS];
    uint8_t outReg[G2_MAX_OUT]; int32_t outWidth[G2_MAX_OUT], outString[G2_MAX_OUT], outSrcCap[G2_MAX_OUT];
};
// ... 6 lines not shown
    GenericSinkDesc sink{};
    int nRegs = 0;
    GenericInstr* dCode = nullptr; GenericProbeDesc* dProbes = nullptr; char* dConstPool = nullptr;
};
struct GenericTableRef { uint32_t* state; void* words; void* acc; uint64_t cap; uint32_t* count; int nWords; };
struct GenericPipelineLaunch {
    const GenericProgram2* prog; const GenericInstr* dCode; const GenericProbeDesc* dProbes; const char* dConstPool;
    GenericTableRef tables[G2_MAX_TABLES];
    int64_t nRows, row0;
    uint32_t* matCnt; const uint64_t* matOffs; uint64_t matLimit; void* matOut[G2_MAX_OUT]; int matPass;
    uint64_t* dense; int64_t denseGroups;
};
void launchGenericPipeline(Context& ctx, const GenericPipelineLaunch& L);
struct Query;
bool buildGenericPlan(Query& q, std::vector<GenericProgram2>& out, std::string& why);

struct Pipeline {
    Table* src = nullptr;
    std::vector<int> cols;
    SinkKind sink = SinkKind::AGGREGATE;
    int buildTable = -1;
    std::string source;
    std::string sourceFlat;
    Kernel* kernelFlat = nullptr;
    std::string sourceCells, sourceFlatCells;
    Kernel* kernelCells = nullptr; Kernel* kernelFlatCells = nullptr;
    std::vector<int> rowCellsEnvelopes;
    int cellsChoice = -1;
    int cellsRuns[2] = {0, 0};
    float cellsBestMs[2] = {0, 0};
    int lastForm = -1;
    int cellsLaunched[2] = {0, 0};
    bool measuring = false; int measureForm = 0;
    std::string sourcePass1;
    Kernel* kernelPass1 = nullptr;
    bool partitioned = false;
    std::string sourcePartCount, sourcePartScatter, sourcePartAgg;
    Kernel* kernelPartCount = nullptr; Kernel* kernelPartScatter = nullptr; Kernel* kernelPartAgg = nullptr;
    std::vector<ArgSlot> argsPartAgg;
    std::vector<int> partRecordInputs;
    int partCount = 0;
    int partGroups = 0;
    int partAtomicsPerRow = 0;
    bool staged = false;
    double leadPass = -1.0;
    bool lateLoads = false;
    int stagedRecWords = 1, stagedRows = 4;
    std::string sourceStagedScatter, sourceStagedAgg;
    Kernel* kernelStagedScatter = nullptr; Kernel* kernelStagedAgg = nullptr;
    std::vector<ArgSlot> argsStagedAgg;
    bool stagedExact = false;
    std::vector<uint32_t> stagedCaps;
    int64_t stagedCapsRows = -1;
    std::string entry = "rsq_pipeline";
    std::vector<ArgSlot> args;
    Kernel* kernel = nullptr;
    int64_t bytesPerRow = 0;
    int64_t storedBytesPerRow = 0;
    bool hasStage2 = false;
    bool compact = false;
    int compactWords = 0;
    int compactWordsLazy = 0;
    int gridPerCULazy = 2;
    std::vector<int> lazyCols;
    std::string sourceLazy;
    Kernel* kernelLazy = nullptr;
// ... 321 lines not shown
```

resql_amd/csrc/engine_pipelines.cpp:

```cpp
#include <algorithm>
#include <atomic>
#include <chrono>
#include <cstring>
#include <sstream>

#include "engine_internal.h"

namespace rsq {

uint64_t argValue(Query& q, const Pipeline& p, const ArgSlot& a, int countOnlyTable) {
    if (a.name == "out") return (uint64_t)(uintptr_t)(q.aggPad > 1 && !q.flatRun ? q.dAggWork : q.dAgg);
    if (a.name == "fin_out") return (uint64_t)(uintptr_t)q.finOut;
    if (a.name == "fin_err") return (uint64_t)(uintptr_t)q.finErr;
    if (a.name == "fin_seq") return q.finOut ? q.finSeq : 0;
    if (a.name == "fin_ticket") return (uint64_t)(uintptr_t)(q.finOut ? q.dFinTicket : nullptr);
    if (a.name == "part_counts") return (uint64_t)(uintptr_t)q.dPartCounts;
    if (a.name == "part_start") return (uint64_t)(uintptr_t)q.dPartStart;
    if (a.name == "tile_step") return (uint64_t)q.partTileStep;
    if (a.name == "rec" || a.name == "sp_rec") return q.dPartRecords.empty() ? 0 : (uint64_t)(uintptr_t)q.dPartRecords[0];
    if (a.name == "dbg") {
        if (!q.dDebugStamps) { q.dDebugStamps = (uint64_t*)q.ctx.alloc(4096 * 8 * 8); RSQ_HIP(hipMemset(q.dDebugStamps, 0, 4096 * 8 * 8)); }
        return (uint64_t)(uintptr_t)q.dDebugStamps;
    }
    if (a.name == "sp_base") return (uint64_t)(uintptr_t)q.dStageBase;
// ... 88 lines not shown
}

unsigned slicedGrid(const Query& q, const Pipeline& p, int64_t want, int64_t cap) {
    const int64_t S = p.nljSliced >= 0 ? std::max<int32_t>(1, q.nljs[(size_t)p.nljSliced].slices) : 1;
    return (unsigned)(S * std::max<int64_t>(1, std::min<int64_t>(want, cap / S)));
}

unsigned pipelineGrid(const Query& q, const Pipeline& p, bool lazyForm) {
    int64_t want, cap;
    pipelineGridLimits(q, p, lazyForm, want, cap);
    return slicedGrid(q, p, want, cap);
}

void prepareRowCellsForm(Query& q, Pipeline& p) {
    p.measuring = false; p.measureForm = 0;
    if (!p.kernelCells || q.ctx.rowCellsMode != -1 || p.cellsChoice >= 0) return;
    if (!rowcells::launchFits(p.rowCellsEnvelopes, (uint64_t)p.src->nRows, pipelineGrid(q, p), (uint64_t)p.blockThreads)) return;
    p.measuring = true;
    if (p.cellsLaunched[0] < 2) return;
    p.measureForm = 1;
    if (p.cellsLaunched[1] < 2) return;
    resolveKernelTime(q);
    if (p.cellsRuns[0] < 2 || p.cellsRuns[1] < 2) return;
    p.cellsChoice = p.cellsBestMs[1] < p.cellsBestMs[0] * (1.0f - kRowCellsMargin) ? 1 : 0;
    p.measuring = false; p.measureForm = 0;
}
void noteRowCellsTime(Query& q, int form, float ms) {
    if (form < 0 || form > 1 || q.pipelines.empty()) return;
    Pipeline& p = q.pipelines[0];
    if (p.cellsChoice >= 0) return;
    if (p.cellsRuns[form] == 0 || ms < p.cellsBestMs[form]) p.cellsBestMs[form] = ms;
    p.cellsRuns[form]++;
}
std::string rowCellsLine(const Query& q) {
    for (auto& p : q.pipelines) {
        if (p.lastForm < 0) continue;
        char b[200];
        const char* why = q.ctx.rowCellsMode == 0 ? "set by the context"
                          : q.ctx.rowCellsMode == 1 ? (p.lastForm ? "set by the context" : "the launch does not fit the fields of a shared word")
                          : p.cellsChoice < 0 ? "not decided yet" : "decided";
        if (p.cellsRuns[0] && p.cellsRuns[1])
            snprintf(b, sizeof b, "aggregation form of the last execution: %s (%s; %u workgroups; best kernel times %.1f us in registers, %.1f us in cells)\n",
                     p.lastForm ? "1, rows into LDS cells" : "0, registers", why, p.lastGrid, p.cellsBestMs[0] * 1000.0, p.cellsBestMs[1] * 1000.0);
        else snprintf(b, sizeof b, "aggregation form of the last execution: %s (%s; %u workgroups)\n", p.lastForm ? "1, rows into LDS cells" : "0, registers", why, p.lastGrid);
        return b;
    }
    return std::string();
}

void launchPipelineKernel(Query& q, Pipeline& p, Kernel& k, int countOnlyTable, unsigned grid, unsigned block) {
    p.lastGrid = grid ? grid : pipelineGrid(q, p);
    Kernel* form = &k;
    p.lastForm = -1;
    if (p.kernelCells && (form == p.kernel || form == p.kernelFlat)) {
        int f = q.ctx.rowCellsMode == 0 ? 0 : q.ctx.rowCellsMode == 1 ? 1 : p.cellsChoice >= 0 ? p.cellsChoice : p.measureForm;
        if (f == 1 && !rowcells::launchFits(p.rowCellsEnvelopes, (uint64_t)p.src->nRows, p.lastGrid, (uint64_t)(block ? block : (unsigned)p.blockThreads))) f = 0;
        Kernel* cells = form == p.kernel ? p.kernelCells : p.kernelFlatCells;
        if (f == 1 && cells) form = cells; else f = 0;
        p.lastForm = f;
    }
    if (p.nljSliced >= 0 && p.lastGrid % (unsigned)std::max<int32_t>(1, q.nljs[(size_t)p.nljSliced].slices) != 0)
        failRuntime("internal error: " + p.entry + " launches " + std::to_string(p.lastGrid) + " workgroups, no multiple of its " +
                    std::to_string(q.nljs[(size_t)p.nljSliced].slices) + " inner-range slices");
    std::vector<uint64_t> args;
    for (auto& a : p.args) args.push_back(argValue(q, p, a, countOnlyTable));
    launch(q.ctx, *form, p.lastGrid, block ? block : (unsigned)p.blockThreads, args);
    q.report.num_kernels++;
}

void waitForStream(Context& ctx) {
    if (sw::flag<sw::RSQ_POLL>()) {
        const double deadline = nowMs() + 2.0;
        for (;;) {
            const hipError_t e = hipStreamQuery(ctx.stream);
            if (e == hipSuccess) { ctx.streamDrained(); return; }
            if (e != hipErrorNotReady) RSQ_HIP(e);
            if (nowMs() > deadline) break;
            __builtin_ia32_pause();
        }
    }
    RSQ_HIP(hipStreamSynchronize(ctx.stream));
    ctx.streamDrained();
}

void debugStamps(Query& q, Pipeline& p) {
    if (!q.dDebugStamps || p.lastGrid == 0 || p.lastGrid > 4096) return;
    bool has = false;
    for (auto& a : p.args) has = has || a.name == "dbg";
    if (!has) return;
    RSQ_HIP(hipStreamSynchronize(q.ctx.stream));
    std::vector<uint64_t> st((size_t)p.lastGrid * 8);
    RSQ_HIP(hipMemcpy(st.data(), q.dDebugStamps, st.size() * 8, hipMemcpyDeviceToHost));
    RSQ_HIP(hipMemset(q.dDebugStamps, 0, st.size() * 8));
    uint64_t t0 = ~0ull;
    for (unsigned w = 0; w < p.lastGrid; w++) if (st[w * 8]) t0 = std::min(t0, st[w * 8]);
    auto dist = [&](int k) {
        std::vector<double> v;
        for (unsigned w = 0; w < p.lastGrid; w++) if (st[w * 8 + k]) v.push_back((double)(st[w * 8 + k] - t0) / 100.0);
// ... 646 lines not shown
```

resql_amd/csrc/kernels/rsq_device.h:

```cpp
#pragma once

typedef long long i64;
typedef unsigned long long u64;
typedef int i32;
typedef unsigned int u32;
typedef unsigned char u8;
typedef unsigned short u16;

#define RSQ_WAVE 64
#define RSQ_TILE_ROWS 128
#define RSQ_DEV __device__ inline __attribute__((always_inline))

namespace rsq {

enum { ERR_DIV_ZERO = 1, ERR_HT_FULL = 2, ERR_DUP_KEY = 4, ERR_GROUP_OVERFLOW = 8, ERR_STUCK = 16,
       NOTE_CHAR_GROUP_ENDS_WITH_SPACE = 32 ,
       NOTE_BUILD_KEYS_NOT_UNIQUE = 64  };

RSQ_DEV i64 add(i64 a, i64 b) { return (i64)((u64)a + (u64)b); }
RSQ_DEV i64 sub(i64 a, i64 b) { return (i64)((u64)a - (u64)b); }
RSQ_DEV i64 mul(i64 a, i64 b) { return (i64)((u64)a * (u64)b); }
RSQ_DEV i64 div(i64 a, i64 b, u32* err) {
    if (b == 0 || (a == (i64)0x8000000000000000ull && b == -1)) { atomicOr(err, (u32)ERR_DIV_ZERO); return 0; }
    return a / b;
}

struct __attribute__((aligned(16))) i64x2 { i64 x, y; };
struct __attribute__((aligned(16))) u64x2 { u64 x, y; };
struct __attribute__((aligned(8))) i32x2 { i32 x, y; };
struct __attribute__((aligned(2))) u8x2 { u8 x, y; };

#ifdef RSQ_NT_LOADS
typedef i64 i64v2 __attribute__((ext_vector_type(2)));
typedef i32 i32v2 __attribute__((ext_vector_type(2)));
RSQ_DEV void ld2(const i64* p, i64 (&v)[2]) { i64v2 t = __builtin_nontemporal_load(reinterpret_cast<const i64v2*>(p)); v[0] = t.x; v[1] = t.y; }
RSQ_DEV void ld2(const i32* p, i32 (&v)[2]) { i32v2 t = __builtin_nontemporal_load(reinterpret_cast<const i32v2*>(p)); v[0] = t.x; v[1] = t.y; }
RSQ_DEV void ld2(const u8* p, u8 (&v)[2]) { u16 t = __builtin_nontemporal_load(reinterpret_cast<const u16*>(p)); v[0] = (u8)(t & 0xff); v[1] = (u8)(t >> 8); }
#else
RSQ_DEV void ld2(const i64* p, i64 (&v)[2]) { i64x2 t = *reinterpret_cast<const i64x2*>(p); v[0] = t.x; v[1] = t.y; }
RSQ_DEV void ld2(const i32* p, i32 (&v)[2]) { i32x2 t = *reinterpret_cast<const i32x2*>(p); v[0] = t.x; v[1] = t.y; }
RSQ_DEV void ld2(const u8* p, u8 (&v)[2]) { u8x2 t = *reinterpret_cast<const u8x2*>(p); v[0] = t.x; v[1] = t.y; }
#endif

template <typename T, typename N> RSQ_DEV T dec(N x, i64 base) { return (T)(i64)((u64)base + (u64)x); }
#ifdef RSQ_NT_LOADS
#define RSQ_LD_NARROW(T, p) __builtin_nontemporal_load(reinterpret_cast<const T*>(p))
#else
#define RSQ_LD_NARROW(T, p) (*reinterpret_cast<const T*>(p))
#endif
typedef u32 u32v2 __attribute__((ext_vector_type(2)));
template <typename T> RSQ_DEV void ld2n(const u8* p, i64 base, T (&v)[2]) { const u32 t = RSQ_LD_NARROW(u16, p); v[0] = dec<T>(t & 0xffu, base); v[1] = dec<T>(t >> 8, base); }
template <typename T> RSQ_DEV void ld2n(const u16* p, i64 base, T (&v)[2]) { const u32 t = RSQ_LD_NARROW(u32, p); v[0] = dec<T>(t & 0xffffu, base); v[1] = dec<T>(t >> 16, base); }
template <typename T> RSQ_DEV void ld2n(const u32* p, i64 base, T (&v)[2]) { const u32v2 t = RSQ_LD_NARROW(u32v2, p); v[0] = dec<T>(t.x, base); v[1] = dec<T>(t.y, base); }

RSQ_DEV u8 dict_bit(const u64* table, u8 code) { return (u8)((table[code >> 6] >> (code & 63u)) & 1ull); }

typedef u32 u32v4 __attribute__((ext_vector_type(4)));
template <int W, int R>
RSQ_DEV u32v4 ld_str_chunk(const char* tile, int lane) {
    int c = R * 64 + lane;
    if ((R + 1) * 64 > 8 * W) c = c < 8 * W ? c : 8 * W - 1;
    return __builtin_nontemporal_load(reinterpret_cast<const u32v4*>(tile) + c);
}
template <int W, int R>
RSQ_DEV void st_str_chunk(char* ldsTile, int lane, u32v4 v) {
    const int c = R * 64 + lane;
    if ((R + 1) * 64 <= 8 * W || c < 8 * W) reinterpret_cast<u32v4*>(ldsTile)[c] = v;
}

RSQ_DEV void wave_lds_order() { asm volatile("" ::: "memory"); }

template <int NW>
RSQ_DEV void flush_tile_records(i64* ldsTile, i64* dst, int lane) {
    wave_lds_order();
    const u32v4* src = reinterpret_cast<const u32v4*>(ldsTile);
    u32v4* out = reinterpret_cast<u32v4*>(dst);
#pragma unroll
    for (int r = 0; r < NW; r++) out[r * 64 + lane] = src[r * 64 + lane];
    wave_lds_order();
}

RSQ_DEV u64 shfl_xor_u64(u64 v, int mask) {
    u32 lo = (u32)v, hi = (u32)(v >> 32);
    lo = (u32)__shfl_xor((int)lo, mask, 64);
    hi = (u32)__shfl_xor((int)hi, mask, 64);
    return ((u64)hi << 32) | lo;
// ... 401 lines not shown
```

resql_amd/csrc/multi.cpp:

```cpp
#include <dlfcn.h>
#include <rccl/rccl.h>

#include <algorithm>
#include <cstring>
#include <set>

#include "engine_internal.h"
#include "shard_exchange.h"

using namespace rsq;

namespace {

struct RcclApi {
    void* handle = nullptr;
    ncclResult_t (*CommInitAll)(ncclComm_t*, int, const int*) = nullptr;
    ncclResult_t (*CommDestroy)(ncclComm_t) = nullptr;
    ncclResult_t (*Reduce)(const void*, void*, size_t, ncclDataType_t, ncclRedOp_t, int, ncclComm_t, hipStream_t) = nullptr;
    ncclResult_t (*GroupStart)() = nullptr;
    ncclResult_t (*GroupEnd)() = nullptr;
    const char* (*GetErrorString)(ncclResult_t) = nullptr;
};

RcclApi& rccl() {
// ... 166 lines not shown
            failUnsupported("table " + name + " is sharded (its shards differ) but is a build side of the nested-loops plan: across GPUs only the "
                            "nested-loops join's outer table and one table of its inner side may be sharded - replicate " + name);
        shardedInner.push_back(o);
    }
    if (shardedInner.size() > 1)
        failUnsupported("the inner side of the nested-loops join reads two sharded tables (" + tab(0, tableOf(shardedInner[0]))->name + ", " +
                        tab(0, tableOf(shardedInner[1]))->name + "): at most one may be sharded - replicate the others");
    if (!shardedInner.empty() && shardedInner[0] != innerScan)
        failUnsupported("table " + tab(0, tableOf(shardedInner[0]))->name + " is sharded but is not the source of the nested-loops join's inner side "
                        "(a build side, or under a nested inner side): replicate it");
    const int gathered = shardedInner.empty() ? -1 : shardedInner[0];
    if (gathered >= 0) {
        const int t = tableOf(gathered);
        for (int op = p.ops[nlj].child[0]; op != gathered; op = pipelineChild(p.ops[op]))
            if (p.ops[op].tag == RSQ_OP_ORDERBY || p.ops[op].tag == RSQ_OP_AGGREGATION)
                failUnsupported("table " + tab(0, t)->name + " is sharded, and the nested-loops join's inner side over it is sorted or aggregated: replicate it");
        for (int i = 1; i < n; i++)
            if (tab(i, t)->row0 < tab(i - 1, t)->row0 + tab(i - 1, t)->nRows)
                failUnsupported("table " + tab(0, t)->name + " is the sharded inner side of a nested-loops join, and its shards must hold increasing row "
                                "ranges (shard " + std::to_string(i) + " starts at row " + std::to_string((long long)tab(i, t)->row0) + ", before the end of shard " +
                                std::to_string(i - 1) + "'s rows): set each shard's first row (rsq_table_set_first_row)");
        *gatheredTable = t;
    } else *gatheredTable = -1;
    return outerScan;
}

std::unique_ptr<Table> sliceOf(const Table& t, int64_t start, int64_t rows) {
    std::unique_ptr<Table> v(new Table());
    v->ctx = t.ctx; v->name = t.name; v->nRows = rows; v->row0 = t.row0 + start; v->nRowsTotal = t.totalRows();
    v->cols = t.cols;
    for (TableColumn& c : v->cols) {
        c.owned = false;
        c.nw = 0; c.nbase = 0; c.nptr = nullptr; c.nbytes = 0;
        c.dictN = 0; c.dict.clear(); c.dictPtr = nullptr; c.codePtr = nullptr; c.codeBytes = 0;
        if (c.dptr) c.dptr = (char*)c.dptr + (size_t)start * (size_t)columnWidth(c.type);
    }
    return v;
}

void executeNestedLoops(rsq_multi_query& mq) {
    rsq_multi& m = *mq.m;
    NljSplit& sp = mq.split;
    const int n = (int)m.ctxs.size();
    std::vector<NljState*> nl((size_t)n);
    int64_t outer = 0;
    for (int i = 0; i < n; i++) { nl[(size_t)i] = &topNestedLoops(*mq.qs[(size_t)i]); outer += nl[(size_t)i]->outerSrc->nRows; }
    std::vector<int64_t> rows((size_t)n, 0);
    onShardThreads(n, [&](int i) {
        RSQ_HIP(hipSetDevice(m.ctxs[(size_t)i]->device));
        runNestedLoopsInner(*nl[(size_t)i], outer > 0);
        rows[(size_t)i] = nl[(size_t)i]->nInner;
        sp.innerDone[(size_t)i].record(m.ctxs[(size_t)i]->stream);
    });
    int64_t inner = 0;
    for (int i = 0; i < n; i++) {
        if (!sp.gathered && rows[(size_t)i] != rows[0])
            throw Error(RSQ_ERR_RUNTIME, "internal: replicated inner sides of a nested-loops join differ between shards (" + std::to_string((long long)rows[0]) +
                                         " and " + std::to_string((long long)rows[(size_t)i]) + " rows)");
        inner = sp.gathered ? inner + rows[(size_t)i] : rows[0];
    }
    try {
        for (int i = 0; i < n; i++) { RSQ_HIP(hipSetDevice(m.ctxs[(size_t)i]->device)); bindNestedLoops(*mq.qs[(size_t)i], *nl[(size_t)i], outer, inner); }
    } catch (const Error&) {
        mq.report = rsq_report{};
        for (int i = 0; i < n; i++) { mq.report.num_kernels += (int32_t)nl[(size_t)i]->sub.kernels; mq.report.bytes_read += nl[(size_t)i]->sub.bytes; }
        throw;
// ... 358 lines not shown
```

resql_amd/csrc/runtime.cpp:

```cpp
#include "engine.h"
#include "kernel_compile_options.h"

#include <dlfcn.h>
#include <hip/hip_ext.h>
#include <hip/hiprtc.h>
#include <signal.h>
#include <spawn.h>
#include <sys/stat.h>
#include <sys/wait.h>
#include <unistd.h>

#include <chrono>
#include <cstdio>
#include <cstring>
#include <atomic>
#include <fstream>
#include <sstream>
#include <thread>

extern char** environ;

namespace rsq {

static std::string libraryDir() {
// ... 198 lines not shown
}
void Context::freePinned(void* p) {
    if (!p) return;
    if (pinArena && pinArena->free(p)) { if (pinArena->freeBytes() > ((size_t)1 << 30)) pinArena->trim((size_t)256 << 20); return; }
    if (pinNcArena && pinNcArena->free(p)) { if (pinNcArena->freeBytes() > ((size_t)1 << 30)) pinNcArena->trim((size_t)256 << 20); return; }
    allocStats.rawCalls++;
    StopWatch raw(allocStats.rawMs);
    (void)hipHostFree(p);
}

void Table::bumpVersion() {
    version++;
    if (ctx) ctx->retireKeyIndexes(uid);
}
void Context::retireKeyIndexes(uint64_t uid) {
    for (auto it = keyIndexes.begin(); it != keyIndexes.end();) {
        if (it->second.uid != uid) { ++it; continue; }
        it->second.retired = true;
        if (it->second.refs <= 0) { if (it->second.dBitmap) free(it->second.dBitmap); it = keyIndexes.erase(it); } else ++it;
    }
}
void Context::releaseKeyIndex(KeyIndex* k) {
    if (!k || --k->refs > 0 || !k->retired) return;
    for (auto it = keyIndexes.begin(); it != keyIndexes.end(); ++it)
        if (&it->second == k) { if (k->dBitmap) free(k->dBitmap); keyIndexes.erase(it); return; }
}

Table::~Table() {
    if (ctx) ctx->retireKeyIndexes(uid);
    if (ctx && ctx->device >= 0) {
        for (auto& c : cols) {
            if (c.owned && c.dptr) ctx->freeRaw(c.dptr);
            if (c.owned && c.nptr) { ctx->freeRaw(c.nptr); ctx->columnImageBytes -= c.nbytes; }
            if (c.owned && c.dictPtr) { ctx->freeRaw(c.dictPtr); ctx->columnImageBytes -= 256ull * (uint64_t)columnWidth(c.type) + 16; }
            if (c.owned && c.codePtr) { ctx->freeRaw(c.codePtr); ctx->columnImageBytes -= c.codeBytes; }
        }
    } else {
        for (auto& c : cols) if (c.owned && c.dptr) ::free(c.dptr);
    }
}

static bool readFile(const std::string& path, std::string& out) {
    std::ifstream f(path, std::ios::binary);
    if (!f.is_open()) return false;
    std::ostringstream ss; ss << f.rdbuf();
    out = ss.str();
    return true;
}

static const char* const kHiprtcArch = RSQ_HIPRTC_ARCH;
static const char* const kHiprtcOpt = RSQ_HIPRTC_OPT;
static const char* const kHiprtcStd = RSQ_HIPRTC_STD;

static std::string compileWithHiprtc(Context& ctx, const std::string& source) {
    hiprtcProgram prog;
    if (hiprtcCreateProgram(&prog, source.c_str(), "rsq_pipeline.hip", 0, nullptr, nullptr) != HIPRTC_SUCCESS)
        throw Error(RSQ_ERR_DEVICE, "hiprtcCreateProgram failed");
    std::string inc = "-I" + ctx.includeDir;
    const char* opts[] = {kHiprtcArch, kHiprtcOpt, kHiprtcStd, inc.c_str()};
    hiprtcResult r = hiprtcCompileProgram(prog, 4, opts);
    if (r != HIPRTC_SUCCESS) {
        size_t n = 0; hiprtcGetProgramLogSize(prog, &n);
        std::string log(n, '\0');
        if (n) hiprtcGetProgramLog(prog, &log[0]);
        hiprtcDestroyProgram(&prog);
        throw Error(RSQ_ERR_DEVICE, "hiprtc compilation failed:\n" + log);
// ... 156 lines not shown
```

resql_amd/engine.py:

```python
from __future__ import annotations

import ctypes as C
import os
from typing import List, Optional, Sequence

import numpy as np

from . import plan as P

_HERE = os.path.dirname(os.path.abspath(__file__))
LIB_PATH = os.path.join(_HERE, "libresql_hip.so")

STATUS = {0: "OK", 1: "INVALID", 2: "TYPE", 3: "UNSUPPORTED", 4: "DEVICE", 5: "RUNTIME", 6: "NOMEM"}


class rsq_config(C.Structure):
    _fields_ = [("struct_size", C.c_uint32),
                ("print_assembly", C.c_int32), ("print_flounder", C.c_int32), ("print_performance", C.c_int32),
                ("num_threads", C.c_int32), ("emit_machine_code", C.c_int32), ("optimize", C.c_int32),
                ("device", C.c_int32), ("kernel_cache_dir", C.c_char_p), ("emission_order", C.c_int32),
                ("compat_flags", C.c_uint32), ("engine_flags", C.c_uint32), ("reserved0", C.c_uint32),
                ("arena_reserve_bytes", C.c_int64), ("arena_keep_bytes", C.c_int64), ("nested_loops_max_pairs", C.c_int64),
                ("nested_loops_inner_slices", C.c_int32), ("tbl_ingest", C.c_int32)]

# ... 156 lines not shown
        L.rsq_table_total_rows.argtypes = [vp]
        L.rsq_table_destroy.argtypes = [vp]
        L.rsq_query_compile.argtypes = [vp, C.POINTER(P.rsq_plan_desc), C.POINTER(vp), i32, C.POINTER(vp)]
        L.rsq_query_execute.argtypes = [vp]
        L.rsq_query_await_kernels.argtypes = [vp]
        L.rsq_query_execute_partial.argtypes = [vp, C.POINTER(vp), C.POINTER(i64), C.POINTER(i64), C.POINTER(i64)]
        L.rsq_query_execute_partial_async.argtypes = [vp]
        L.rsq_ctx_set_stream.argtypes = [vp, vp, i32]
        L.rsq_query_finalize.argtypes = [vp]
        L.rsq_query_bind_partial.argtypes = [vp, vp, C.c_size_t]
        L.rsq_query_merge_gathered.argtypes = [vp, vp, i32]
        L.rsq_query_finalize_host.argtypes = [vp, C.POINTER(i64), i64]
        L.rsq_query_partial_layout.argtypes = [vp, C.POINTER(i64), C.POINTER(i64), C.POINTER(i64)]
        L.rsq_query_result.argtypes = [vp, C.POINTER(P.rsq_result_view)]
        L.rsq_query_report.argtypes = [vp, C.POINTER(rsq_report)]
        L.rsq_query_kernel_time_stats.argtypes = [vp, C.POINTER(C.c_double), C.POINTER(C.c_uint64), C.c_int32]
        L.rsq_query_nested_loops_slices.argtypes = [vp, C.POINTER(i32)]
        L.rsq_nested_loops_slices.restype = i32
        L.rsq_nested_loops_slices.argtypes = [i64, i64, i64, i32]
        L.rsq_query_source.restype = C.c_char_p
        L.rsq_query_source.argtypes = [vp]
        L.rsq_query_explain.restype = C.c_char_p
        L.rsq_query_explain.argtypes = [vp]
        L.rsq_query_destroy.argtypes = [vp]
        L.rsq_serialize_expr.restype = vp
        L.rsq_serialize_expr.argtypes = [vp, C.POINTER(P.rsq_plan_desc), i32, i32, C.POINTER(vp), i32]
        L.rsq_result_serialize.restype = vp
        L.rsq_result_serialize.argtypes = [C.POINTER(P.rsq_result_view)]
        L.rsq_free.argtypes = [vp]
        L.rsq_query_result_text.argtypes = [vp, C.POINTER(rsq_result_text_options), C.POINTER(rsq_result_text_report), C.POINTER(vp), C.POINTER(i64)]
        L.rsq_query_result_write.argtypes = [vp, C.c_char_p, C.POINTER(rsq_result_text_options), C.POINTER(rsq_result_text_report)]
        L.rsq_ctx_set_result_text.argtypes = [vp, i32]
        L.rsq_ctx_set_row_cells.argtypes = [vp, i32]
        L.rsq_db_result_text_report.argtypes = [vp, C.POINTER(rsq_result_text_report)]
        L.rsq_ctx_set_order_limit.argtypes = [vp, i32]
        L.rsq_query_order_limit_report.argtypes = [vp, C.POINTER(rsq_order_limit_report)]
        L.rsq_db_order_limit_report.argtypes = [vp, C.POINTER(rsq_order_limit_report)]
        L.rsq_prim_column_topk.argtypes = [vp, vp, i32, i64, i32, i64, i64, vp, i32, vp, vp, vp, vp, vp]
        L.rsq_ref_emission_order.argtypes = [vp, i64, C.c_uint64, i32, vp]
        L.rsq_ref_emission_order_device.argtypes = [vp, vp, i64, C.c_uint64, vp]
        L.rsq_prim_exclusive_scan.argtypes = [vp, vp, i64, i32, vp, vp]
        L.rsq_prim_rank_index.argtypes = [vp, vp, i64, i32, vp, vp]
        L.rsq_prim_rank_place.argtypes = [vp, vp, i64, i64, i64, vp, vp, i32, i32, i32, i64, vp, vp]
        L.rsq_prim_radix_sort_pairs.argtypes = [vp, vp, vp, i64, i32, vp, vp, vp]
        L.rsq_prim_running_min.argtypes = [vp, vp, i64, vp, vp]
        L.rsq_prim_merge_group_rows.argtypes = [vp, vp, i64, i32, i32, vp, vp, vp, i32, vp, vp, i32, vp, vp, vp]
        L.rsq_prim_topk_select.argtypes = [vp, vp, i64, i64, i32, i32, i32, i32, i64, i32, vp, i64, vp, vp, vp]
        L.rsq_measure_read_bandwidth.argtypes = [vp, C.c_size_t, i32, C.POINTER(C.c_double)]
        L.rsq_sql_plan_select.argtypes = [vp, C.c_char_p, C.POINTER(vp), i32, C.POINTER(vp)]
        L.rsq_sql_plan_desc.restype = C.POINTER(P.rsq_plan_desc)
        L.rsq_sql_plan_desc.argtypes = [vp]
        L.rsq_sql_plan_destroy.argtypes = [vp]
        L.rsq_sql_plan_text.restype = vp
        L.rsq_sql_plan_text.argtypes = [vp]
        L.rsq_sql_compile.argtypes = [vp, C.c_char_p, C.POINTER(vp), i32, C.POINTER(vp)]
        L.rsq_sql_describe.restype = vp
        L.rsq_sql_describe.argtypes = [vp, C.c_char_p, i32]
        L.rsq_db_create.argtypes = [vp, C.POINTER(vp)]
        L.rsq_db_execute.argtypes = [vp, C.c_char_p, C.POINTER(i32), C.POINTER(P.rsq_result_view)]
        L.rsq_db_adopt_table.argtypes = [vp, vp]
        L.rsq_db_message.restype = C.c_char_p
        L.rsq_db_message.argtypes = [vp]
        L.rsq_db_report.argtypes = [vp, C.POINTER(rsq_report)]
        L.rsq_db_load_report.argtypes = [vp, C.POINTER(rsq_tbl_load_report)]
        L.rsq_db_destroy.argtypes = [vp]
        L.rsq_multi_create.argtypes = [C.POINTER(rsq_multi_config), C.POINTER(vp)]
# ... 2 lines not shown
        L.rsq_multi_last_error.argtypes = [vp]
        L.rsq_multi_devices.restype = i32
        L.rsq_multi_devices.argtypes = [vp]
        L.rsq_multi_ctx.restype = vp
        L.rsq_multi_ctx.argtypes = [vp, i32]
        L.rsq_multi_merge_name.restype = C.c_char_p
        L.rsq_multi_merge_name.argtypes = [vp]
        L.rsq_multi_shard_rows.restype = None
        L.rsq_multi_shard_rows.argtypes = [i64, i32, i32, C.POINTER(i64), C.POINTER(i64)]
        L.rsq_multi_table_generate.argtypes = [vp, i32, i64, C.c_double, i64, C.c_uint64, C.POINTER(vp)]
        L.rsq_multi_table_generate_on_key.argtypes = [vp, i32, i64, C.c_double, i64, C.c_uint64, C.c_char_p, C.POINTER(vp)]
        L.rsq_multi_query_merge_name.restype = C.c_char_p
        L.rsq_multi_query_merge_name.argtypes = [vp]
        L.rsq_multi_query_explain.restype = C.c_char_p
        L.rsq_multi_query_explain.argtypes = [vp, i32]
        L.rsq_multi_query_compile.argtypes = [vp, C.POINTER(P.rsq_plan_desc), C.POINTER(vp), i32, C.POINTER(vp)]
        L.rsq_multi_query_execute.argtypes = [vp]
        L.rsq_multi_query_result.argtypes = [vp, C.POINTER(P.rsq_result_view)]
        L.rsq_multi_query_report.argtypes = [vp, C.POINTER(rsq_report), C.POINTER(C.c_double)]
        L.rsq_multi_query_collective_ms.restype = C.c_double
        L.rsq_multi_query_collective_ms.argtypes = [vp]
        L.rsq_multi_query_destroy.argtypes = [vp]
        _lib = L
    return _lib


EXPORTED_SYMBOLS = [
    "rsq_ctx_create", "rsq_ctx_destroy", "rsq_last_error", "rsq_table_create", "rsq_table_create_device",
    "rsq_table_from_rowstore", "rsq_table_from_rowstore_ex", "rsq_ctx_set_rowstore_bridge", "rsq_table_load_tbl", "rsq_table_load_tbl_ex", "rsq_table_generate", "rsq_table_rows", "rsq_table_set_first_row", "rsq_table_refresh_stats", "rsq_table_append", "rsq_ctx_memory_stats", "rsq_table_read_column", "rsq_table_read_image",
    "rsq_table_stats_bytes", "rsq_table_stats_export", "rsq_table_unify_shard_stats", "rsq_table_unify_shard_dictionaries", "rsq_table_time_dictionary_pass", "rsq_table_total_rows",
    "rsq_table_destroy", "rsq_query_compile", "rsq_query_execute", "rsq_query_await_kernels", "rsq_query_execute_partial",
    "rsq_query_execute_partial_async", "rsq_ctx_set_stream",
    "rsq_query_finalize", "rsq_query_merge_gathered", "rsq_query_finalize_host", "rsq_query_bind_partial", "rsq_query_partial_layout", "rsq_query_result", "rsq_query_report", "rsq_query_kernel_time_stats", "rsq_query_nested_loops_slices", "rsq_nested_loops_slices", "rsq_query_source", "rsq_query_explain",
    "rsq_query_destroy", "rsq_serialize_expr", "rsq_result_serialize", "rsq_free", "rsq_query_result_text", "rsq_query_result_write", "rsq_ctx_set_result_text", "rsq_ctx_set_row_cells", "rsq_db_result_text_report", "rsq_ref_emission_order", "rsq_ref_emission_order_device",
    "rsq_prim_exclusive_scan", "rsq_prim_rank_index", "rsq_prim_rank_place",
    "rsq_prim_radix_sort_pairs", "rsq_prim_running_min", "rsq_prim_merge_group_rows", "rsq_prim_topk_select", "rsq_prim_column_topk",
    "rsq_ctx_set_order_limit", "rsq_query_order_limit_report", "rsq_db_order_limit_report",
    "rsq_measure_read_bandwidth",
    "rsq_sql_plan_select", "rsq_sql_plan_desc", "rsq_sql_plan_destroy", "rsq_sql_plan_text", "rsq_sql_compile", "rsq_sql_describe",
    "rsq_db_create", "rsq_db_execute", "rsq_db_message", "rsq_db_adopt_table", "rsq_db_report", "rsq_db_load_report", "rsq_db_destroy",
    "rsq_multi_create", "rsq_multi_destroy", "rsq_multi_last_error", "rsq_multi_devices", "rsq_multi_ctx", "rsq_multi_merge_name",
    "rsq_multi_shard_rows", "rsq_multi_table_generate", "rsq_multi_table_generate_on_key", "rsq_multi_query_merge_name", "rsq_multi_query_explain", "rsq_multi_query_compile", "rsq_multi_query_execute",
    "rsq_multi_query_result", "rsq_multi_query_report", "rsq_multi_query_collective_ms", "rsq_multi_query_destroy",
]

NLJ_MIN_SLICE_ROWS = 512


def nested_loops_slices(base_workgroups: int, max_workgroups: int, inner_rows: int, configured: int = 0) -> int:
    return lib().rsq_nested_loops_slices(base_workgroups, max_workgroups, inner_rows, configured)


def unify_shard_dictionaries(tables: Sequence["DeviceTable"]) -> None:
    if not tables:
        raise ValueError("unify_shard_dictionaries: no tables")
    arr = (C.c_void_p * len(tables))(*[t.h for t in tables])
    tables[0].ctx._check(lib().rsq_table_unify_shard_dictionaries(arr, len(tables)))


GEN_LINEITEM, GEN_ORDERS, GEN_CUSTOMER, GEN_SYNTHETIC = 0, 1, 2, 3
RANK_CHUNK_BLOCKS = 1024


class Context:

    @classmethod
    def borrowed(cls, handle, device: int) -> "Context":
# ... 91 lines not shown
                         rows_upper_bound: Optional[int] = None, image_range=None):
        rows = np.ascontiguousarray(rows, dtype=np.int64)
        n, stride = rows.shape
        rng = None if image_range is None else np.array([int(x) & 0xffffffffffffffff for x in image_range], dtype=np.uint64)
        cand = np.zeros((capacity, stride), dtype=np.int64)
        count, notes = C.c_uint32(0xffffffff), C.c_uint32(0xffffffff)
        self._check(self._L.rsq_prim_topk_select(self.h, rows.ctypes.data, n, n if rows_upper_bound is None else rows_upper_bound, stride, key_word,
                                                 1 if is32 else 0, 1 if desc else 0, want, form, None if rng is None else rng.ctypes.data, capacity,
                                                 cand.ctypes.data, C.addressof(count), C.addressof(notes)))
        return cand, count.value, notes.value

    def prim_column_topk(self, key: np.ndarray, desc: bool, want: int, capacity: int, payload: np.ndarray):
        key = np.ascontiguousarray(key)
        if key.dtype not in (np.dtype(np.int32), np.dtype(np.int64)):
            raise ValueError("prim_column_topk: the key column is int32 or int64")
        payload = np.ascontiguousarray(payload, dtype=np.uint8).reshape(len(key), -1)
        width = payload.shape[1]
        positions = np.zeros(capacity, dtype=np.uint32)
        out = np.zeros((capacity, width), dtype=np.uint8)
        count, threshold, notes = C.c_uint64(0xffffffffffffffff), C.c_uint64(0), C.c_uint32(0xffffffff)
        self._check(self._L.rsq_prim_column_topk(self.h, key.ctypes.data, key.dtype.itemsize, len(key), 1 if desc else 0, want, capacity,
                                                 payload.ctypes.data, width, positions.ctypes.data, out.ctypes.data, C.addressof(count),
                                                 C.addressof(threshold), C.addressof(notes)))
        return positions, out, count.value, threshold.value, notes.value

    def set_order_limit(self, where: int):
        self._check(self._L.rsq_ctx_set_order_limit(self.h, where))

    def set_result_text(self, where: int):
        self._check(self._L.rsq_ctx_set_result_text(self.h, where))

    def set_row_cells(self, mode: int):
        self._check(self._L.rsq_ctx_set_row_cells(self.h, mode))

    def set_rowstore_bridge(self, where: int):
        self._check(self._L.rsq_ctx_set_rowstore_bridge(self.h, where))

    def set_stream(self, hip_stream: Optional[int]):
        self._check(self._L.rsq_ctx_set_stream(self.h, hip_stream or None, 0 if hip_stream is None else 1))

    def _adopt(self, child):
        import weakref
        if not hasattr(self, "_children"):
            self._children = weakref.WeakSet()
        self._children.add(child)

    def close(self):
        if getattr(self, "h", None):
            for child in list(getattr(self, "_children", ())):
                try:
                    child.close()
                except Exception:
                    pass
            if not getattr(self, "_borrowed", False):
                self._L.rsq_ctx_destroy(self.h)
            self.h = None

    def __del__(self):
        try:
            self.close()
        except Exception:
            pass

    def table(self, t: P.Table) -> "DeviceTable":
        keep: list = []
        d = t.to_c(keep)
# ... 158 lines not shown
    def unify_shard_stats(self, blobs: Sequence[bytes]):
        joined = b"".join(blobs)
        self.ctx._check(self.ctx._L.rsq_table_unify_shard_stats(self.h, joined, len(blobs), len(blobs[0]) if blobs else 0))

    def time_dictionary_pass(self, name: str, which: int) -> float:
        ms = C.c_double(0)
        self.ctx._check(self.ctx._L.rsq_table_time_dictionary_pass(self.h, name.encode(), which, C.byref(ms)))
        return ms.value

    def read_column(self, name: str, dtype, count: Optional[int] = None) -> np.ndarray:
        n = self.n_rows if count is None else count
        out = np.empty(n, dtype=dtype)
        self.ctx._check(self.ctx._L.rsq_table_read_column(self.ctx.h, self.h, name.encode(), out.ctypes.data, out.nbytes))
        return out

    def image_info(self, name: str) -> tuple:
        info = (C.c_int64 * 4)()
        self.ctx._check(self.ctx._L.rsq_table_read_image(self.ctx.h, self.h, name.encode(), 0, None, 0, info))
        return tuple(int(v) for v in info)

    def read_image(self, name: str, which: int) -> np.ndarray:
        if which not in (0, 1, 2):
            raise ValueError("read_image: which is 0 (narrow image), 1 (dictionary entries) or 2 (dictionary codes)")
        width, _, entries, rows = self.image_info(name)
        if which == 1 and entries and name not in self.widths:
            raise KeyError(f"read_image: the width of column {name} is not known to this handle")
        n = (rows * width, entries * self.widths.get(name, 0), rows if entries else 0)[which]
        out = np.empty(n, dtype=np.uint8)
        if n:
            info = (C.c_int64 * 4)()
            self.ctx._check(self.ctx._L.rsq_table_read_image(self.ctx.h, self.h, name.encode(), which, out.ctypes.data, n, info))
        return out

    def close(self):
        if self.h:
            self.ctx._L.rsq_table_destroy(self.h)
            self.h = None


class Query:
    def __init__(self, ctx: Context, h):
        self.ctx, self.h = ctx, h
        ctx._adopt(self)

    def execute(self):
        self.ctx._check(self.ctx._L.rsq_query_execute(self.h))

    def await_kernels(self):
        self.ctx._check(self.ctx._L.rsq_query_await_kernels(self.h))

    def execute_partial(self):
        p = C.c_void_p(); a = C.c_int64(); b = C.c_int64(); c = C.c_int64()
        self.ctx._check(self.ctx._L.rsq_query_execute_partial(self.h, C.byref(p), C.byref(a), C.byref(b), C.byref(c)))
        return p.value, a.value, b.value, c.value

    def execute_partial_async(self):
        self.ctx._check(self.ctx._L.rsq_query_execute_partial_async(self.h))

    def finalize_host(self, words: np.ndarray):
        w = np.ascontiguousarray(words, dtype=np.int64)
        self.ctx._check(self.ctx._L.rsq_query_finalize_host(self.h, w.ctypes.data_as(C.POINTER(C.c_int64)), w.size))

    def bind_partial(self, dev_ptr: int, nbytes: int):
        self.ctx._check(self.ctx._L.rsq_query_bind_partial(self.h, dev_ptr, nbytes))

    def merge_gathered(self, gathered_dev_ptr: int, n_ranks: int):
# ... 249 lines not shown
```

Baseline: 488.1 billion rows/s.

## Add nibble-plane column images with a second plane-based scan form

Adds bit-plane encodings of narrow-range integer, decimal and date columns, split into a low plane and an optional high plane at 4, 12, 20 or 24 bits per value. They are built on device next to the existing byte images. Codegen emits a second scan form that decodes values from the planes, with the aim of cutting scanned bytes per row on bandwidth-bound scans such as Q1. In exchange it adds extra device memory, an encode kernel at table load, two-form kernel generation, and extra decode arithmetic per row.

```diff
diff --git a/__graft_entry__.py b/__graft_entry__.py
--- a/__graft_entry__.py
+++ b/__graft_entry__.py
@@ -159,6 +159,25 @@
                     finally:
                         for k in list(env) + ["RSQ_DICT_SCANS"]:
                             os.environ.pop(k, None)
+        elif kind == "plane":
+            import planecases
+            for i, plan in enumerate(planecases.warm_plans()):
+                if i not in items:
+                    continue
+                for planes, cells in ((1, 1), (1, 0), (0, 0)):
+                    ctx.set_plane_scan(planes)
+                    ctx.set_row_cells(cells)
+                    try:
+                        tabs = [ctx.table(t) for t in plan.tables]
+                        ctx.compile(plan, tabs).close()
+                        for t in tabs:
+                            t.close()
+                        done += 1
+                    except engine.EngineError as e:
+                        failed += e.status not in (2, 3)
+                    finally:
+                        ctx.set_plane_scan(-1)
+                        ctx.set_row_cells(-1)
         elif kind == "resulttext":
             import resulttextcases
             for i, (sql, host) in enumerate(resulttextcases.warm_statements()):
@@ -205,7 +224,8 @@
                         ("dictgroup", list(range(64))),
                         ("dicttail", list(range(32))),
                         ("dictjoin", list(range(32))),
-                        ("resulttext", list(range(32)))):
+                        ("resulttext", list(range(32))),
+                        ("plane", list(range(16)))):
         for i in range(n):
             part = seeds[i::n]
             if part:
diff --git a/include/resql_hip.h b/include/resql_hip.h
--- a/include/resql_hip.h
+++ b/include/resql_hip.h
@@ -193,6 +193,8 @@
 int  rsq_query_result_write(rsq_query* q, const char* path, const rsq_result_text_options* options, rsq_result_text_report* report);
 int  rsq_ctx_set_result_text(rsq_ctx* ctx, int32_t where);
 int  rsq_ctx_set_row_cells(rsq_ctx* ctx, int32_t mode);
+int  rsq_ctx_set_plane_scan(rsq_ctx* ctx, int32_t mode);
+int  rsq_ctx_plane_image_bytes(const rsq_ctx* ctx, uint64_t* bytes);
 int  rsq_ctx_set_order_limit(rsq_ctx* ctx, int32_t where);
 enum rsq_order_limit_fallback { RSQ_ORDER_LIMIT_FALLBACK_NONE = 0, RSQ_ORDER_LIMIT_FALLBACK_SHAPE = 1, RSQ_ORDER_LIMIT_FALLBACK_FEW_ROWS = 2,
                                 RSQ_ORDER_LIMIT_FALLBACK_OVERFLOW = 3, RSQ_ORDER_LIMIT_FALLBACK_TIES = 4 };
@@ -232,6 +234,7 @@
                            uint32_t* positions_out , void* payload_out , uint64_t* cand_count,
                            uint64_t* threshold_image, uint32_t* notes);
 int   rsq_table_read_image(rsq_ctx* ctx, const rsq_table* t, const char* column, int32_t which, void* host_dst, size_t bytes, int64_t info[4]);
+int   rsq_table_read_planes(rsq_ctx* ctx, const rsq_table* t, const char* column, int32_t which, void* host_dst, size_t bytes, int64_t info[4]);
 
 typedef struct rsq_sql_plan rsq_sql_plan;
 int  rsq_sql_plan_select(rsq_ctx* ctx, const char* sql, rsq_table* const* tables, int32_t n_tables, rsq_sql_plan** out);
diff --git a/integration/resql_hip_binding.h b/integration/resql_hip_binding.h
--- a/integration/resql_hip_binding.h
+++ b/integration/resql_hip_binding.h
@@ -176,6 +176,8 @@
 
     void setRowstoreBridge(int where) { check(rsq_ctx_set_rowstore_bridge(ctx_, where)); }
     void setOrderLimit(int where) { check(rsq_ctx_set_order_limit(ctx_, where)); }
+    void setPlaneScan(int mode) { check(rsq_ctx_set_plane_scan(ctx_, mode)); }
+    uint64_t planeImageBytes() { uint64_t b = 0; check(rsq_ctx_plane_image_bytes(ctx_, &b)); return b; }
 
     int64_t bulkInsert(Relation* rel, const std::string& name, const std::string& fileName, char fieldTerminator) {
         std::vector<rsq_column> cols = columnsOf(rel);
diff --git a/resql_amd/csrc/aot_kernels.hip b/resql_amd/csrc/aot_kernels.hip
--- a/resql_amd/csrc/aot_kernels.hip
+++ b/resql_amd/csrc/aot_kernels.hip
@@ -4,6 +4,7 @@
 #include <cstring>
 
 #include "engine_internal.h"
+#include "plane_image.h"
 #include "scan_device.h"
 
 namespace rsq {
@@ -87,6 +88,15 @@
     const int w = range <= 0xffull ? 1 : range <= 0xffffull ? 2 : range <= 0xffffffffull ? 4 : 0;
     if (tag == RSQ_INT && w != 1) return 0;
     return w > 0 && w < columnWidth(c.type) ? w : 0;
+}
+
+int planeWidthOf(const TableColumn& c) {
+    if (!sw::flag<sw::RSQ_NARROW_SCANS>()) return 0;
+    if (!c.owned || !c.dptr || !c.stats.valid || c.type.isString()) return 0;
+    const int tag = c.type.tag;
+    if (tag != RSQ_INT && tag != RSQ_BIGINT && tag != RSQ_DECIMAL && tag != RSQ_DATE) return 0;
+    if (c.stats.min == INT64_MIN || c.stats.max == INT64_MAX || c.stats.max < c.stats.min) return 0;
+    return plane::planeWidth((uint64_t)c.stats.max - (uint64_t)c.stats.min, narrowWidth(c), columnWidth(c.type), tag == RSQ_INT);
 }
 
 enum { DICT_MAX = 256, DICT_SLOTS = 1024, DICT_SAMPLE_ROWS = 65536, DICT_COLLECT_GRID = 512 };
@@ -416,6 +426,57 @@
     return (double)ms;
 }
 
+template <typename T, int BITS>
+__global__ void __launch_bounds__(256) k_encode_planes(const T* __restrict__ src, unsigned char* __restrict__ lo, unsigned char* __restrict__ hi, i64 n, i64 base) {
+    const int LB = plane::lowBits(BITS), HB = plane::highBits(BITS);
+    const i64 pairs = (n + 1) >> 1;
+    for (i64 p = blockIdx.x * (i64)blockDim.x + threadIdx.x; p < pairs; p += (i64)gridDim.x * blockDim.x) {
+        const i64 r = p * 2;
+        const unsigned x0 = plane::imageOf((i64)src[r], base);
+        const unsigned x1 = r + 1 < n ? plane::imageOf((i64)src[r + 1], base) : 0u;
+        const unsigned l0 = plane::lowOf(x0, BITS), l1 = plane::lowOf(x1, BITS);
+        if (LB == 4) lo[p] = (unsigned char)(l0 | l1 << 4);
+        else if (LB == 8) reinterpret_cast<unsigned short*>(lo)[p] = (unsigned short)(l0 | l1 << 8);
+        else reinterpret_cast<unsigned*>(lo)[p] = l0 | l1 << 16;
+        const unsigned h0 = plane::highOf(x0, BITS), h1 = plane::highOf(x1, BITS);
+        if (HB == 4) hi[p] = (unsigned char)(h0 | h1 << 4);
+        else if (HB == 8) reinterpret_cast<unsigned short*>(hi)[p] = (unsigned short)(h0 | h1 << 8);
+    }
+}
+
+template <typename T>
+static void launchEncodePlanes(Context& ctx, const TableColumn& c, i64 n) {
+    const unsigned grid = 1024;
+    unsigned char* lo = (unsigned char*)c.plo; unsigned char* hi = (unsigned char*)c.phi;
+    if (c.pbits == 4) hipLaunchKernelGGL((k_encode_planes<T, 4>), dim3(grid), dim3(256), 0, ctx.stream, (const T*)c.dptr, lo, hi, n, (i64)c.pbase);
+    else if (c.pbits == 12) hipLaunchKernelGGL((k_encode_planes<T, 12>), dim3(grid), dim3(256), 0, ctx.stream, (const T*)c.dptr, lo, hi, n, (i64)c.pbase);
+    else if (c.pbits == 20) hipLaunchKernelGGL((k_encode_planes<T, 20>), dim3(grid), dim3(256), 0, ctx.stream, (const T*)c.dptr, lo, hi, n, (i64)c.pbase);
+    else hipLaunchKernelGGL((k_encode_planes<T, 24>), dim3(grid), dim3(256), 0, ctx.stream, (const T*)c.dptr, lo, hi, n, (i64)c.pbase);
+}
+
+static bool buildPlaneImage(Context& ctx, Table& t, TableColumn& c, bool& launched) {
+    const int bits = t.nRows > 0 && ctx.planeScans() ? planeWidthOf(c) : 0;
+    const int64_t base = bits ? c.stats.min : 0;
+    const size_t loBytes = plane::lowPlaneBytes(t.nRows, bits), hiBytes = plane::highPlaneBytes(t.nRows, bits);
+    const bool keep = ctx.device >= 0 && c.plo && bits == c.pbits && base == c.pbase && loBytes == c.ploBytes && hiBytes == c.phiBytes;
+    bool moved = false;
+    if (!keep && c.plo) {
+        if (ctx.device >= 0) { ctx.freeRaw(c.plo); ctx.planeImageBytes -= c.ploBytes; if (c.phi) { ctx.freeRaw(c.phi); ctx.planeImageBytes -= c.phiBytes; } }
+        c.plo = c.phi = nullptr; moved = true;
+    }
+    c.pbits = bits; c.pbase = base; c.ploBytes = loBytes; c.phiBytes = hiBytes;
+    if (!bits || ctx.device < 0) return moved;
+    if (!c.plo) {
+        c.plo = ctx.allocRaw(loBytes); ctx.planeImageBytes += loBytes;
+        if (hiBytes) { c.phi = ctx.allocRaw(hiBytes); ctx.planeImageBytes += hiBytes; }
+    }
+    launched = true;
+    if (c.type.tag == RSQ_INT) launchEncodePlanes<int>(ctx, c, (i64)t.nRows);
+    else if (c.type.tag == RSQ_DATE) launchEncodePlanes<unsigned>(ctx, c, (i64)t.nRows);
+    else launchEncodePlanes<i64>(ctx, c, (i64)t.nRows);
+    return moved;
+}
+
 template <typename T, typename N>
 __global__ void __launch_bounds__(256) k_encode(const T* __restrict__ src, N* __restrict__ dst, i64 n, i64 base) {
     for (i64 i = blockIdx.x * (i64)blockDim.x + threadIdx.x; i < n; i += (i64)gridDim.x * blockDim.x)
@@ -433,6 +494,7 @@
 static void buildNarrowImages(Context& ctx, Table& t) {
     bool moved = false, launched = false;
     for (auto& c : t.cols) {
+        moved = buildPlaneImage(ctx, t, c, launched) || moved;
         const int w = t.nRows > 0 ? narrowWidth(c) : 0;
         const int64_t base = w ? c.stats.min : 0;
         const size_t bytes = w ? (((size_t)t.nRows * (size_t)w + 15) & ~(size_t)15) : 0;
diff --git a/resql_amd/csrc/api.cpp b/resql_amd/csrc/api.cpp
--- a/resql_amd/csrc/api.cpp
+++ b/resql_amd/csrc/api.cpp
@@ -461,6 +461,39 @@
         if (!src) failInvalid("the column has no such image");
         RSQ_HIP(hipStreamSynchronize(C(ctx)->stream));
         RSQ_HIP(hipMemcpy(host_dst, src, bytes, hipMemcpyDeviceToHost));
+    });
+}
+
+int rsq_table_read_planes(rsq_ctx* ctx, const rsq_table* t, const char* name, int32_t which, void* host_dst, size_t bytes, int64_t info[4]) {
+    if (!ctx || !t || !name || !info || which < 0 || which > 1 || (bytes && !host_dst)) return RSQ_ERR_INVALID;
+    return guarded(C(ctx), [&] {
+        const Table* tb = reinterpret_cast<const Table*>(t);
+        if (tb->ctx != C(ctx)) failInvalid("the table belongs to another context");
+        int ci = tb->findCol(name);
+        if (ci < 0) failInvalid(std::string("no such column: ") + name);
+        const TableColumn& c = tb->cols[(size_t)ci];
+        info[0] = c.pbits; info[1] = c.pbits ? c.pbase : 0; info[2] = (int64_t)c.ploBytes; info[3] = (int64_t)c.phiBytes;
+        if (!bytes) return;
+        if (C(ctx)->device < 0) failUnsupported("a compile-only context keeps no plane image");
+        if (bytes > (which == 0 ? c.ploBytes : c.phiBytes)) failInvalid("read beyond the plane");
+        const void* src = which == 0 ? c.plo : c.phi;
+        if (!src) failInvalid("the column has no such plane");
+        RSQ_HIP(hipStreamSynchronize(C(ctx)->stream));
+        RSQ_HIP(hipMemcpy(host_dst, src, bytes, hipMemcpyDeviceToHost));
+    });
+}
+
+int rsq_ctx_plane_image_bytes(const rsq_ctx* ctx, uint64_t* out) {
+    if (!ctx || !out) return RSQ_ERR_INVALID;
+    *out = reinterpret_cast<const Context*>(ctx)->planeImageBytes;
+    return RSQ_OK;
+}
+
+int rsq_ctx_set_plane_scan(rsq_ctx* ctx, int32_t mode) {
+    if (!ctx) return RSQ_ERR_INVALID;
+    return guarded(C(ctx), [&] {
+        if (mode < -1 || mode > 1) failInvalid("plane_scan is " + std::to_string(mode) + " (-1: the default rule, 0: no plane images and no second scan form, 1: wherever a statement and its table have them)");
+        C(ctx)->planeScanMode = mode;
     });
 }
 
diff --git a/resql_amd/csrc/codegen.cpp b/resql_amd/csrc/codegen.cpp
--- a/resql_amd/csrc/codegen.cpp
+++ b/resql_amd/csrc/codegen.cpp
@@ -1,11 +1,12 @@
 #include "codegen_internal.h"
+#include "plane_image.h"
 
 namespace rsq {
 namespace cg {
 
-void Walker::addArg(const std::string& name, const std::string& ctype, uint64_t v) {
+void Walker::addArg(const std::string& name, const std::string& ctype, uint64_t v, bool plane) {
     for (auto& a : pipe.args) if (a.name == name) return;
-    pipe.args.push_back({name, ctype, v});
+    pipe.args.push_back({name, ctype, v, plane});
 }
 
 void Walker::produce(OpNode* o, std::vector<std::string> request) {
@@ -207,7 +208,7 @@
     pipe.unroll = 1;
     pipe.blockThreads = 256;
     pipe.maxGrid = q.maxGrid;
-    colTypes.clear(); colIsString.clear(); colNarrow.clear(); colDict.clear(); colTyped.clear(); eg.typedLeaves.clear(); nDictTables = 0; rowParams.clear(); rowArgsTail.clear(); rowArgsTailGuarded.clear(); bitmapPrefetch.clear();
+    colTypes.clear(); colIsString.clear(); colNarrow.clear(); colPlane.clear(); colDict.clear(); colTyped.clear(); eg.typedLeaves.clear(); nDictTables = 0; rowParams.clear(); rowArgsTail.clear(); rowArgsTailGuarded.clear(); bitmapPrefetch.clear();
     body.clear(); stateDecl.clear(); stateInit.clear(); prologue.clear(); epilogue.clear(); fileScope.clear(); helperFns.clear();
     explainSteps.clear(); indent = 1; matchSlotTable = -1; slotVar.clear(); symbolOrigin.clear(); symbolWord.clear();
     multiMatchAbove = false; repeatedKeysAbove.clear(); denseRefusal.clear();
@@ -234,9 +235,13 @@
         pipe.bytesPerRow += columnWidth(c.type);
         const int nw = (!t->derived && c.owned && narrowScans && !c.type.isString() && (c.nptr || q.ctx.device < 0)) ? c.nw : 0;
         colNarrow.push_back(nw);
+        const int pb = (!t->derived && c.owned && narrowScans && !c.type.isString() && q.ctx.planeScans() && (c.plo || q.ctx.device < 0)) ? c.pbits : 0;
+        colPlane.push_back(pb);
         const bool dictCoded = !t->derived && c.owned && c.type.isString() && c.dictN > 0 && sw::dictScansEnabled() && (c.codePtr || q.ctx.device < 0);
         colDict.push_back(dictCoded ? c.type.len : 0);
         pipe.storedBytesPerRow += dictCoded ? 1 : nw ? nw : columnWidth(c.type);
+        pipe.planeHalfBytesPerRow += pb ? plane::halfBytesPerRow(pb) : 2 * (dictCoded ? 1 : nw ? nw : columnWidth(c.type));
+        if (pb) pipe.planeForm = true;
         if (dictCoded) {
             const std::string K = std::to_string(k);
             addArg("c" + K, "const u8*", (uint64_t)(uintptr_t)c.codePtr);
@@ -258,6 +263,11 @@
                 addArg("c" + std::to_string(k), std::string("const ") + (nw == 1 ? "u8" : nw == 2 ? "u16" : "u32") + "*", (uint64_t)(uintptr_t)c.nptr);
                 addArg("fb" + std::to_string(k), "i64", (uint64_t)c.nbase);
             } else addArg("c" + std::to_string(k), "const " + ct + "*", (uint64_t)(uintptr_t)c.dptr);
+            if (pb) {
+                addArg("pl" + std::to_string(k), "const u8*", (uint64_t)(uintptr_t)c.plo, true);
+                if (plane::highBits(pb)) addArg("ph" + std::to_string(k), "const u8*", (uint64_t)(uintptr_t)c.phi, true);
+                if (!nw) addArg("fb" + std::to_string(k), "i64", (uint64_t)c.pbase, true);
+            }
             colIsString.push_back(0); colTypes.push_back(ct);
             rowParams += ", " + ct + " " + var;
             rowArgsTail += ", " + colAt(k, "r");
@@ -266,7 +276,8 @@
     }
     explainSteps.push_back("scan " + t->name + " [" + (t->derived ? std::string("rows of this execution") : std::to_string((long long)t->nRows) + " rows") + ", " +
                            std::to_string((long long)pipe.bytesPerRow) + " B/row" +
-                           (pipe.storedBytesPerRow != pipe.bytesPerRow ? ", " + std::to_string((long long)pipe.storedBytesPerRow) + " B/row stored" : std::string()) + "]");
+                           (pipe.storedBytesPerRow != pipe.bytesPerRow ? ", " + std::to_string((long long)pipe.storedBytesPerRow) + " B/row stored" : std::string()) + "]" +
+                           (pipe.planeForm ? " [plane images: " + std::to_string((long long)(pipe.planeHalfBytesPerRow / 2)) + (pipe.planeHalfBytesPerRow & 1 ? ".5" : "") + " B/row stored]" : std::string()));
     consume(o->parent, o);
     finishPipeline();
 }
diff --git a/resql_amd/csrc/codegen_agg.cpp b/resql_amd/csrc/codegen_agg.cpp
--- a/resql_amd/csrc/codegen_agg.cpp
+++ b/resql_amd/csrc/codegen_agg.cpp
@@ -740,6 +740,7 @@
         patch(rowParams, ", i64 v_" + K, ", i32 n_" + K);
         patch(rowArgsTail, "rsq::dec<i64>(a.c" + K + "[", "rsq::dec<i32>(a.c" + K + "[");
         patch(rowArgsTailGuarded, "rsq::dec<i64>(a.c" + K + "[", "rsq::dec<i32>(a.c" + K + "[");
+        for (std::string* text : {&rowArgsTail, &rowArgsTailGuarded}) patch(*text, ", i64>(a.pl" + K + ",", ", i32>(a.pl" + K + ",");
         colTyped[k] = 1; colTypes[k] = "i32";
         eg.typedLeaves["v_" + K] = ExprGen::TypedLeaf{"n_" + K, neg, bits};
         widen += "    const i64 v_" + K + " = (i64)n_" + K + "; (void)v_" + K + ";\n";
diff --git a/resql_amd/csrc/codegen_internal.h b/resql_amd/csrc/codegen_internal.h
--- a/resql_amd/csrc/codegen_internal.h
+++ b/resql_amd/csrc/codegen_internal.h
@@ -314,14 +314,27 @@
     std::vector<int> colNarrow;
     std::string colAt(int k, const std::string& r) const {
         const std::string K = std::to_string(k);
-        if (k < (int)colNarrow.size() && colNarrow[(size_t)k]) return "rsq::dec<" + colTypes[(size_t)k] + ">(a.c" + K + "[" + r + "], a.fb" + K + ")";
-        return "a.c" + K + "[" + r + "]";
+        const std::string bytes = k < (int)colNarrow.size() && colNarrow[(size_t)k] ? "rsq::dec<" + colTypes[(size_t)k] + ">(a.c" + K + "[" + r + "], a.fb" + K + ")"
+                                                                                    : "a.c" + K + "[" + r + "]";
+        if (!planeCol(k)) return bytes;
+        return twoForms(bytes, "rsq::decp<" + std::to_string(colPlane[(size_t)k]) + ", " + colTypes[(size_t)k] + ">(" + planePtrs(k) + ", " + r + ", a.fb" + K + ")");
     }
     std::string tileLoad(int k, const std::string& dst) const {
         const std::string K = std::to_string(k);
-        if (k < (int)colNarrow.size() && colNarrow[(size_t)k]) return "rsq::ld2n(a.c" + K + " + b, a.fb" + K + ", " + dst + ");";
-        return "rsq::ld2(a.c" + K + " + b, " + dst + ");";
-    }
+        const std::string bytes = k < (int)colNarrow.size() && colNarrow[(size_t)k] ? "rsq::ld2n(a.c" + K + " + b, a.fb" + K + ", " + dst + ");"
+                                                                                    : "rsq::ld2(a.c" + K + " + b, " + dst + ");";
+        if (!planeCol(k)) return bytes;
+        return twoForms(bytes, "rsq::ld2n<" + std::to_string(colPlane[(size_t)k]) + ">(" + planePtrs(k) + ", b, a.fb" + K + ", " + dst + ");");
+    }
+    std::vector<int> colPlane;
+    bool planeCol(int k) const { return k >= 0 && k < (int)colPlane.size() && colPlane[(size_t)k] != 0; }
+    std::string planePtrs(int k) const {
+        const std::string K = std::to_string(k);
+        return "a.pl" + K + ", " + (colPlane[(size_t)k] == 4 ? std::string("nullptr") : "a.ph" + K);
+    }
+    static constexpr char PF_OPEN = '\x02', PF_MID = '\x03', PF_CLOSE = '\x04';
+    static std::string twoForms(const std::string& bytes, const std::string& planes) { return PF_OPEN + bytes + PF_MID + planes + PF_CLOSE; }
+    static std::string resolvePlaneForm(const std::string& text, bool keep);
     std::vector<int> colDict;
     std::vector<char> colTyped;
     bool typedCol(int k) const { return k >= 0 && k < (int)colTyped.size() && colTyped[(size_t)k] != 0; }
@@ -373,7 +386,7 @@
     void line(const std::string& s) { body += std::string((size_t)indent * 4, ' ') + s + "\n"; }
     void openScope(const std::string& head) { line(head); indent++; }
     void closeScope() { indent--; line("}"); }
-    void addArg(const std::string& name, const std::string& ctype, uint64_t v);
+    void addArg(const std::string& name, const std::string& ctype, uint64_t v, bool plane = false);
 
     void produce(OpNode* o, std::vector<std::string> request);
 
diff --git a/resql_amd/csrc/codegen_loop.cpp b/resql_amd/csrc/codegen_loop.cpp
--- a/resql_amd/csrc/codegen_loop.cpp
+++ b/resql_amd/csrc/codegen_loop.cpp
@@ -65,8 +65,39 @@
     text = out;
 }
 
+std::string Walker::resolvePlaneForm(const std::string& text, bool keep) {
+    std::string out, runPlane, runBytes;
+    auto flush = [&]() {
+        if (runBytes.empty()) return;
+        out += keep ? "#if RSQ_PLANE_SCAN\n" + runPlane + "#else\n" + runBytes + "#endif\n" : runBytes;
+        runPlane.clear(); runBytes.clear();
+    };
+    for (size_t at = 0; at < text.size();) {
+        size_t end = text.find('\n', at);
+        end = end == std::string::npos ? text.size() : end + 1;
+        const std::string ln = text.substr(at, end - at);
+        at = end;
+        if (ln.find(PF_OPEN) == std::string::npos) { flush(); out += ln; continue; }
+        int part = 0;
+        for (char ch : ln) {
+            if (ch == PF_OPEN) part = 1;
+            else if (ch == PF_MID) part = 2;
+            else if (ch == PF_CLOSE) part = 0;
+            else { if (part != 2) runBytes += ch; if (part != 1) runPlane += ch; }
+        }
+    }
+    flush();
+    return out;
+}
+
 void Walker::finishPipeline() {
     while (indent > 1) closeScope();
+    const bool hadPlaneColumns = pipe.planeForm;
+    pipe.planeForm = pipe.planeForm && pipe.sink != SinkKind::MATERIALIZE;
+    if (hadPlaneColumns && !pipe.planeForm) {
+        for (auto it = pipe.args.begin(); it != pipe.args.end();) it = it->plane ? pipe.args.erase(it) : it + 1;
+        for (auto& step : explainSteps) { const size_t at = step.find(" [plane images: "); if (at != std::string::npos) step.erase(at); }
+    }
     addArg("n_rows", "i64", (uint64_t)pipe.src->nRows);
     addArg("row0", "i64", (uint64_t)pipe.src->row0);
     addArg("err", "u32*", (uint64_t)(uintptr_t)q.ctx.dErr);
@@ -171,7 +202,12 @@
     s << "#ifndef RSQ_BLOCK_THREADS\n#define RSQ_BLOCK_THREADS " << pipe.blockThreads << "\n#endif\n";
     if (fourWaves) s << "#define RSQ_MIN_WG 4\n";
     s << "struct Args {\n";
-    for (auto& a : pipe.args) s << "    " << a.ctype << " " << a.name << ";\n";
+    for (auto& a : pipe.args) if (!a.plane) s << "    " << a.ctype << " " << a.name << ";\n";
+    if (pipe.planeForm) {
+        s << "#if RSQ_PLANE_SCAN\n";
+        for (auto& a : pipe.args) if (a.plane) s << "    " << a.ctype << " " << a.name << ";\n";
+        s << "#endif\n";
+    }
     s << "};\nstruct State {\n" << stateDecl << "};\n";
     s << helperFns;
     if (cq) {
@@ -503,7 +539,7 @@
     s << epilogue;
     if (dbgStamps) s << "    __syncthreads();\n    if (a.dbg && threadIdx.x == 0) a.dbg[(u64)blockIdx.x * 8 + 3] = (u64)wall_clock64();\n";
     s << "}\n";
-    pipe.source = s.str();
+    pipe.source = hadPlaneColumns ? resolvePlaneForm(s.str(), pipe.planeForm) : s.str();
     if (!pipe.lazyCols.empty()) pipe.source = "#define RSQ_LAZY 0\n" + pipe.source;
     if (mat) {
         pipe.sourcePass1 = "#define RSQ_PASS 1\n" + pipe.source;
diff --git a/resql_amd/csrc/engine.cpp b/resql_amd/csrc/engine.cpp
--- a/resql_amd/csrc/engine.cpp
+++ b/resql_amd/csrc/engine.cpp
@@ -229,6 +229,8 @@
         v.push_back(T(p.source));
         if (!p.sourceCells.empty()) v.push_back(T(p.sourceCells));
         if (!p.sourceFlatCells.empty()) v.push_back(T(p.sourceFlatCells));
+        if (p.planeForm)
+            for (const std::string* s : {&p.source, &p.sourceFlat, &p.sourceCells, &p.sourceFlatCells, &p.sourceLazy}) if (!s->empty()) v.push_back(T(Pipeline::planeSource(*s)));
         if (!p.sourceLazy.empty()) v.push_back(T(p.sourceLazy));
         if (p.ldsSlots > 64 && q.aggMode == AggMode::HASH && p.sink == SinkKind::AGGREGATE && q.aggTable >= 0) {
             v.push_back(T("#define RSQ_LC_SLOTS 64\n" + p.source));
@@ -258,6 +260,12 @@
         p.kernel = &ctx.getKernel(T(p.source), p.entry);
         if (!p.sourceCells.empty()) p.kernelCells = &ctx.getKernel(T(p.sourceCells), p.entry);
         if (!p.sourceFlatCells.empty()) p.kernelFlatCells = &ctx.getKernel(T(p.sourceFlatCells), p.entry);
+        if (p.planeForm) {
+            int i = 0;
+            for (const std::string* s : {&p.source, &p.sourceFlat, &p.sourceCells, &p.sourceFlatCells, &p.sourceLazy}) {
+                p.kernelPlane[i++] = s->empty() ? nullptr : &ctx.getKernel(T(Pipeline::planeSource(*s)), p.entry);
+            }
+        }
         if (!p.sourceLazy.empty()) p.kernelLazy = &ctx.getKernel(T(p.sourceLazy), p.entry);
         if (ctx.device < 0 && p.ldsSlots > 64 && q.aggMode == AggMode::HASH && p.sink == SinkKind::AGGREGATE && q.aggTable >= 0) {
             (void)ctx.getKernel("#define RSQ_LC_SLOTS 64\n" + p.source, p.entry);
diff --git a/resql_amd/csrc/engine.h b/resql_amd/csrc/engine.h
--- a/resql_amd/csrc/engine.h
+++ b/resql_amd/csrc/engine.h
@@ -52,6 +52,11 @@
     int64_t nbase = 0;
     void* nptr = nullptr;
     size_t nbytes = 0;
+    int pbits = 0;
+    int64_t pbase = 0;
+    void* plo = nullptr;
+    void* phi = nullptr;
+    size_t ploBytes = 0, phiBytes = 0;
     int dictN = 0;
     std::vector<uint8_t> dict;
     void* dictPtr = nullptr;
@@ -61,6 +66,7 @@
 };
 
 int narrowWidth(const TableColumn& c);
+int planeWidthOf(const TableColumn& c);
 
 struct Context;
 
@@ -163,6 +169,10 @@
     void retireKeyIndexes(uint64_t uid);
     void releaseKeyIndex(KeyIndex* k);
     uint64_t columnImageBytes = 0;
+    uint64_t planeImageBytes = 0;
+    int planeScanMode = -1;
+    bool planeScans() const { return planeScanMode == 1 || (planeScanMode == -1 && kPlaneScanDefault); }
+    static constexpr bool kPlaneScanDefault = false;
     uint64_t planMemoClock = 0, planMemoHits = 0;
     bool planMemoOff = false;
     int rowCellsMode = -1;
diff --git a/resql_amd/csrc/engine_internal.h b/resql_amd/csrc/engine_internal.h
--- a/resql_amd/csrc/engine_internal.h
+++ b/resql_amd/csrc/engine_internal.h
@@ -112,7 +112,7 @@
 enum class AggMode { NONE, DENSE_REG, DENSE_LDS_PRIVATE, DENSE_LDS_SHARED, DENSE_GLOBAL, AT_JOIN_ENTRY, HASH };
 enum class SinkKind { AGGREGATE, BUILD, MATERIALIZE };
 
-struct ArgSlot { std::string name; std::string ctype; uint64_t value; };
+struct ArgSlot { std::string name; std::string ctype; uint64_t value; bool plane = false; };
 
 struct GenericInstr { uint8_t op, dst, a, b; uint32_t c; int64_t imm; };
 enum GenericOp : uint8_t { G_COL = 1, G_CONST, G_ADD, G_SUB, G_MUL, G_DIV, G_LT, G_LE, G_GT, G_GE, G_EQ, G_NE, G_AND, G_OR, G_MULI, G_DIVI,
@@ -185,6 +185,11 @@
     int lastForm = -1;
     int cellsLaunched[2] = {0, 0};
     bool measuring = false; int measureForm = 0;
+    bool planeForm = false;
+    int64_t planeHalfBytesPerRow = 0;
+    Kernel* kernelPlane[5] = {nullptr, nullptr, nullptr, nullptr, nullptr};
+    int lastPlane = -1;
+    static std::string planeSource(const std::string& s) { return "#define RSQ_PLANE_SCAN 1\n" + s; }
     std::string sourcePass1;
     Kernel* kernelPass1 = nullptr;
     bool partitioned = false;
diff --git a/resql_amd/csrc/engine_pipelines.cpp b/resql_amd/csrc/engine_pipelines.cpp
--- a/resql_amd/csrc/engine_pipelines.cpp
+++ b/resql_amd/csrc/engine_pipelines.cpp
@@ -144,7 +144,21 @@
     if (p.cellsRuns[form] == 0 || ms < p.cellsBestMs[form]) p.cellsBestMs[form] = ms;
     p.cellsRuns[form]++;
 }
-std::string rowCellsLine(const Query& q) {
+static std::string scanFormLines(const Query& q) {
+    std::string o;
+    for (auto& p : q.pipelines) {
+        if (p.lastPlane < 0) continue;
+        char b[200];
+        if (p.lastPlane) snprintf(b, sizeof b, "scan form of the last execution: %s from plane images (%lld%s B/row)\n", p.entry.c_str(), (long long)(p.planeHalfBytesPerRow / 2), p.planeHalfBytesPerRow & 1 ? ".5" : "");
+        else snprintf(b, sizeof b, "scan form of the last execution: %s from byte images (%lld B/row; %s)\n", p.entry.c_str(), (long long)p.storedBytesPerRow,
+                      q.ctx.planeScans() ? "this launch's kernel has no plane form" : "set by the context");
+        o += b;
+    }
+    return o;
+}
+static std::string aggregationFormLine(const Query& q);
+std::string rowCellsLine(const Query& q) { return aggregationFormLine(q) + scanFormLines(q); }
+static std::string aggregationFormLine(const Query& q) {
     for (auto& p : q.pipelines) {
         if (p.lastForm < 0) continue;
         char b[200];
@@ -171,11 +185,21 @@
         if (f == 1 && cells) form = cells; else f = 0;
         p.lastForm = f;
     }
+    bool planes = false;
+    p.lastPlane = -1;
+    if (p.planeForm) {
+        const int i = form == p.kernel ? 0 : form == p.kernelFlat ? 1 : form == p.kernelCells ? 2 : form == p.kernelFlatCells ? 3 : form == p.kernelLazy ? 4 : -1;
+        planes = i >= 0 && p.kernelPlane[i] && q.ctx.planeScans();
+        for (auto& a : p.args) if (a.plane && a.ctype != "i64" && !a.value) planes = false;
+        if (planes) form = p.kernelPlane[i];
+        p.lastPlane = planes ? 1 : 0;
+    }
     if (p.nljSliced >= 0 && p.lastGrid % (unsigned)std::max<int32_t>(1, q.nljs[(size_t)p.nljSliced].slices) != 0)
         failRuntime("internal error: " + p.entry + " launches " + std::to_string(p.lastGrid) + " workgroups, no multiple of its " +
                     std::to_string(q.nljs[(size_t)p.nljSliced].slices) + " inner-range slices");
     std::vector<uint64_t> args;
-    for (auto& a : p.args) args.push_back(argValue(q, p, a, countOnlyTable));
+    for (auto& a : p.args) if (!a.plane) args.push_back(argValue(q, p, a, countOnlyTable));
+    if (planes) for (auto& a : p.args) if (a.plane) args.push_back(a.value);
     launch(q.ctx, *form, p.lastGrid, block ? block : (unsigned)p.blockThreads, args);
     q.report.num_kernels++;
 }
diff --git a/resql_amd/csrc/kernels/rsq_device.h b/resql_amd/csrc/kernels/rsq_device.h
--- a/resql_amd/csrc/kernels/rsq_device.h
+++ b/resql_amd/csrc/kernels/rsq_device.h
@@ -52,6 +52,32 @@
 template <typename T> RSQ_DEV void ld2n(const u8* p, i64 base, T (&v)[2]) { const u32 t = RSQ_LD_NARROW(u16, p); v[0] = dec<T>(t & 0xffu, base); v[1] = dec<T>(t >> 8, base); }
 template <typename T> RSQ_DEV void ld2n(const u16* p, i64 base, T (&v)[2]) { const u32 t = RSQ_LD_NARROW(u32, p); v[0] = dec<T>(t & 0xffffu, base); v[1] = dec<T>(t >> 16, base); }
 template <typename T> RSQ_DEV void ld2n(const u32* p, i64 base, T (&v)[2]) { const u32v2 t = RSQ_LD_NARROW(u32v2, p); v[0] = dec<T>(t.x, base); v[1] = dec<T>(t.y, base); }
+template <int BITS, typename T> RSQ_DEV void ld2n(const u8* lo, const u8* hi, i64 b, i64 base, T (&v)[2]) {
+    static_assert(BITS == 4 || BITS == 12 || BITS == 20 || BITS == 24, "plane images are 4, 12, 20 or 24 bits wide");
+    u32 x0, x1;
+    if (BITS == 4) { const u32 t = RSQ_LD_NARROW(u8, lo + (b >> 1)); x0 = t & 0xfu; x1 = t >> 4; }
+    else if (BITS == 12) {
+        const u32 t = RSQ_LD_NARROW(u16, lo + b), h = RSQ_LD_NARROW(u8, hi + (b >> 1));
+        x0 = (t & 0xffu) | (h & 0xfu) << 8; x1 = (t >> 8) | (h >> 4) << 8;
+    } else if (BITS == 20) {
+        const u32 t = RSQ_LD_NARROW(u32, lo + b * 2), h = RSQ_LD_NARROW(u8, hi + (b >> 1));
+        x0 = (t & 0xffffu) | (h & 0xfu) << 16; x1 = (t >> 16) | (h >> 4) << 16;
+    } else {
+        const u32 t = RSQ_LD_NARROW(u32, lo + b * 2), h = RSQ_LD_NARROW(u16, hi + b);
+        x0 = (t & 0xffffu) | (h & 0xffu) << 16; x1 = (t >> 16) | (h >> 8) << 16;
+    }
+    v[0] = dec<T>(x0, base); v[1] = dec<T>(x1, base);
+}
+template <int BITS, typename T> RSQ_DEV T decp(const u8* lo, const u8* hi, i64 r, i64 base) {
+    static_assert(BITS == 4 || BITS == 12 || BITS == 20 || BITS == 24, "plane images are 4, 12, 20 or 24 bits wide");
+    const u32 sh = ((u32)r & 1u) * 4u;
+    u32 x;
+    if (BITS == 4) x = ((u32)lo[r >> 1] >> sh) & 0xfu;
+    else if (BITS == 12) x = (u32)lo[r] | (((u32)hi[r >> 1] >> sh) & 0xfu) << 8;
+    else if (BITS == 20) x = (u32)reinterpret_cast<const u16*>(lo)[r] | (((u32)hi[r >> 1] >> sh) & 0xfu) << 16;
+    else x = (u32)reinterpret_cast<const u16*>(lo)[r] | (u32)hi[r] << 16;
+    return dec<T>(x, base);
+}
 
 RSQ_DEV u8 dict_bit(const u64* table, u8 code) { return (u8)((table[code >> 6] >> (code & 63u)) & 1ull); }
 
diff --git a/resql_amd/csrc/multi.cpp b/resql_amd/csrc/multi.cpp
--- a/resql_amd/csrc/multi.cpp
+++ b/resql_amd/csrc/multi.cpp
@@ -222,6 +222,7 @@
     for (TableColumn& c : v->cols) {
         c.owned = false;
         c.nw = 0; c.nbase = 0; c.nptr = nullptr; c.nbytes = 0;
+        c.pbits = 0; c.pbase = 0; c.plo = c.phi = nullptr; c.ploBytes = c.phiBytes = 0;
         c.dictN = 0; c.dict.clear(); c.dictPtr = nullptr; c.codePtr = nullptr; c.codeBytes = 0;
         if (c.dptr) c.dptr = (char*)c.dptr + (size_t)start * (size_t)columnWidth(c.type);
     }
diff --git a/resql_amd/csrc/plane_image.h b/resql_amd/csrc/plane_image.h
--- /dev/null
+++ b/resql_amd/csrc/plane_image.h
@@ -0,0 +1,71 @@
+#pragma once
+#include <cstddef>
+#include <cstdint>
+
+#if defined(__HIPCC__) || defined(__CUDACC__)
+#define RSQ_PLANE_HD __host__ __device__ inline
+#else
+#define RSQ_PLANE_HD inline
+#endif
+
+namespace rsq {
+namespace plane {
+
+RSQ_PLANE_HD int lowBits(int bits) { return bits == 4 ? 4 : bits == 12 ? 8 : bits == 20 || bits == 24 ? 16 : 0; }
+RSQ_PLANE_HD int highBits(int bits) { return bits == 12 || bits == 20 ? 4 : bits == 24 ? 8 : 0; }
+RSQ_PLANE_HD bool isPlaneWidth(int bits) { return lowBits(bits) != 0; }
+
+RSQ_PLANE_HD int bitsForRange(uint64_t range) {
+    return range <= 0xfull ? 4 : range <= 0xffull ? 8 : range <= 0xfffull ? 12 : range <= 0xffffull ? 16 : range <= 0xfffffull ? 20
+         : range <= 0xffffffull ? 24 : range <= 0xffffffffull ? 32 : 0;
+}
+RSQ_PLANE_HD int planeWidth(uint64_t range, int byteImageBytes, int columnBytes, bool narrowInt) {
+    const int bits = bitsForRange(range);
+    if (!isPlaneWidth(bits)) return 0;
+    if (narrowInt && (byteImageBytes != 1 || bits != 4)) return 0;
+    const int readBits = 8 * (byteImageBytes ? byteImageBytes : columnBytes);
+    return bits < readBits ? bits : 0;
+}
+
+RSQ_PLANE_HD size_t planeBytes(int64_t nRows, int cellBits) {
+    if (nRows <= 0 || cellBits == 0) return 0;
+    const size_t b = cellBits == 4 ? ((size_t)nRows + 1) / 2 : (size_t)nRows * (size_t)(cellBits / 8);
+    return (b + 15) & ~(size_t)15;
+}
+RSQ_PLANE_HD size_t lowPlaneBytes(int64_t nRows, int bits) { return planeBytes(nRows, lowBits(bits)); }
+RSQ_PLANE_HD size_t highPlaneBytes(int64_t nRows, int bits) { return planeBytes(nRows, highBits(bits)); }
+RSQ_PLANE_HD int halfBytesPerRow(int bits) { return bits / 4; }
+
+RSQ_PLANE_HD size_t cellByte(int64_t i, int cellBits) { return cellBits == 4 ? (size_t)i >> 1 : (size_t)i * (size_t)(cellBits / 8); }
+RSQ_PLANE_HD int cellShift(int64_t i, int cellBits) { return cellBits == 4 ? (int)(i & 1) * 4 : 0; }
+
+RSQ_PLANE_HD uint32_t getCell(const unsigned char* p, int64_t i, int cellBits) {
+    const unsigned char* b = p + cellByte(i, cellBits);
+    if (cellBits == 4) return (uint32_t)(b[0] >> cellShift(i, 4)) & 0xfu;
+    if (cellBits == 8) return b[0];
+    return (uint32_t)b[0] | (uint32_t)b[1] << 8;
+}
+RSQ_PLANE_HD void putCell(unsigned char* p, int64_t i, int cellBits, uint32_t v) {
+    unsigned char* b = p + cellByte(i, cellBits);
+    if (cellBits == 4) b[0] = (unsigned char)(b[0] | (v & 0xfu) << cellShift(i, 4));
+    else if (cellBits == 8) b[0] = (unsigned char)v;
+    else { b[0] = (unsigned char)v; b[1] = (unsigned char)(v >> 8); }
+}
+
+RSQ_PLANE_HD uint32_t imageOf(int64_t value, int64_t base) { return (uint32_t)((uint64_t)value - (uint64_t)base); }
+RSQ_PLANE_HD uint32_t lowOf(uint32_t image, int bits) { return image & ((1u << lowBits(bits)) - 1u); }
+RSQ_PLANE_HD uint32_t highOf(uint32_t image, int bits) { return image >> lowBits(bits); }
+
+RSQ_PLANE_HD void pack(unsigned char* lo, unsigned char* hi, int64_t i, int bits, int64_t value, int64_t base) {
+    const uint32_t x = imageOf(value, base);
+    putCell(lo, i, lowBits(bits), lowOf(x, bits));
+    if (highBits(bits)) putCell(hi, i, highBits(bits), highOf(x, bits));
+}
+RSQ_PLANE_HD int64_t unpack(const unsigned char* lo, const unsigned char* hi, int64_t i, int bits, int64_t base) {
+    uint32_t x = getCell(lo, i, lowBits(bits));
+    if (highBits(bits)) x |= getCell(hi, i, highBits(bits)) << lowBits(bits);
+    return (int64_t)((uint64_t)base + (uint64_t)x);
+}
+
+}
+}
diff --git a/resql_amd/csrc/runtime.cpp b/resql_amd/csrc/runtime.cpp
--- a/resql_amd/csrc/runtime.cpp
+++ b/resql_amd/csrc/runtime.cpp
@@ -254,6 +254,8 @@
         for (auto& c : cols) {
             if (c.owned && c.dptr) ctx->freeRaw(c.dptr);
             if (c.owned && c.nptr) { ctx->freeRaw(c.nptr); ctx->columnImageBytes -= c.nbytes; }
+            if (c.owned && c.plo) { ctx->freeRaw(c.plo); ctx->planeImageBytes -= c.ploBytes; }
+            if (c.owned && c.phi) { ctx->freeRaw(c.phi); ctx->planeImageBytes -= c.phiBytes; }
             if (c.owned && c.dictPtr) { ctx->freeRaw(c.dictPtr); ctx->columnImageBytes -= 256ull * (uint64_t)columnWidth(c.type) + 16; }
             if (c.owned && c.codePtr) { ctx->freeRaw(c.codePtr); ctx->columnImageBytes -= c.codeBytes; }
         }
diff --git a/resql_amd/engine.py b/resql_amd/engine.py
--- a/resql_amd/engine.py
+++ b/resql_amd/engine.py
@@ -212,6 +212,9 @@
         L.rsq_query_result_write.argtypes = [vp, C.c_char_p, C.POINTER(rsq_result_text_options), C.POINTER(rsq_result_text_report)]
         L.rsq_ctx_set_result_text.argtypes = [vp, i32]
         L.rsq_ctx_set_row_cells.argtypes = [vp, i32]
+        L.rsq_ctx_set_plane_scan.argtypes = [vp, i32]
+        L.rsq_ctx_plane_image_bytes.argtypes = [vp, C.POINTER(C.c_uint64)]
+        L.rsq_table_read_planes.argtypes = [vp, vp, C.c_char_p, i32, vp, C.c_size_t, C.POINTER(i64)]
         L.rsq_db_result_text_report.argtypes = [vp, C.POINTER(rsq_result_text_report)]
         L.rsq_ctx_set_order_limit.argtypes = [vp, i32]
         L.rsq_query_order_limit_report.argtypes = [vp, C.POINTER(rsq_order_limit_report)]
@@ -280,7 +283,7 @@
     "rsq_table_destroy", "rsq_query_compile", "rsq_query_execute", "rsq_query_await_kernels", "rsq_query_execute_partial",
     "rsq_query_execute_partial_async", "rsq_ctx_set_stream",
     "rsq_query_finalize", "rsq_query_merge_gathered", "rsq_query_finalize_host", "rsq_query_bind_partial", "rsq_query_partial_layout", "rsq_query_result", "rsq_query_report", "rsq_query_kernel_time_stats", "rsq_query_nested_loops_slices", "rsq_nested_loops_slices", "rsq_query_source", "rsq_query_explain",
-    "rsq_query_destroy", "rsq_serialize_expr", "rsq_result_serialize", "rsq_free", "rsq_query_result_text", "rsq_query_result_write", "rsq_ctx_set_result_text", "rsq_ctx_set_row_cells", "rsq_db_result_text_report", "rsq_ref_emission_order", "rsq_ref_emission_order_device",
+    "rsq_query_destroy", "rsq_serialize_expr", "rsq_result_serialize", "rsq_free", "rsq_query_result_text", "rsq_query_result_write", "rsq_ctx_set_result_text", "rsq_ctx_set_row_cells", "rsq_ctx_set_plane_scan", "rsq_ctx_plane_image_bytes", "rsq_table_read_planes", "rsq_db_result_text_report", "rsq_ref_emission_order", "rsq_ref_emission_order_device",
     "rsq_prim_exclusive_scan", "rsq_prim_rank_index", "rsq_prim_rank_place",
     "rsq_prim_radix_sort_pairs", "rsq_prim_running_min", "rsq_prim_merge_group_rows", "rsq_prim_topk_select", "rsq_prim_column_topk",
     "rsq_ctx_set_order_limit", "rsq_query_order_limit_report", "rsq_db_order_limit_report",
@@ -438,6 +441,14 @@
 
     def set_row_cells(self, mode: int):
         self._check(self._L.rsq_ctx_set_row_cells(self.h, mode))
+
+    def set_plane_scan(self, mode: int):
+        self._check(self._L.rsq_ctx_set_plane_scan(self.h, mode))
+
+    def plane_image_bytes(self) -> int:
+        v = C.c_uint64(0)
+        self._check(self._L.rsq_ctx_plane_image_bytes(self.h, C.byref(v)))
+        return int(v.value)
 
     def set_rowstore_bridge(self, where: int):
         self._check(self._L.rsq_ctx_set_rowstore_bridge(self.h, where))
@@ -662,6 +673,22 @@
             self.ctx._check(self.ctx._L.rsq_table_read_image(self.ctx.h, self.h, name.encode(), which, out.ctypes.data, n, info))
         return out
 
+    def plane_info(self, name: str) -> tuple:
+        info = (C.c_int64 * 4)()
+        self.ctx._check(self.ctx._L.rsq_table_read_planes(self.ctx.h, self.h, name.encode(), 0, None, 0, info))
+        return tuple(int(v) for v in info)
+
+    def read_planes(self, name: str) -> tuple:
+        _, _, lo, hi = self.plane_info(name)
+        out = []
+        for which, n in ((0, lo), (1, hi)):
+            a = np.empty(n, dtype=np.uint8)
+            if n:
+                info = (C.c_int64 * 4)()
+                self.ctx._check(self.ctx._L.rsq_table_read_planes(self.ctx.h, self.h, name.encode(), which, a.ctypes.data, n, info))
+            out.append(a)
+        return tuple(out)
+
     def close(self):
         if self.h:
             self.ctx._L.rsq_table_destroy(self.h)
```

Result: faster. 497.5 billion rows/s, median of 5 (+1.9%).
